# Fahien/rayca

Hardware: AMD Instinct MI355X
Metric: Mrays/sec (primary+shadow), 1920x1080 Sponza 1spp (higher is better)
Workload: dtype f32; 1 GPU; sponza-STAND-IN procedural atrium 271,568 tris, 1920x1080, primary + 1 shadow ray (Pathtracer max_depth=1, NEE, 1 point light), 1 spp; width=1920, height=1080, triangles=271568, bvh_nodes=135379, bvh_built_on=gpu (bvh_build.hip; same tree as the host builder), rays_per_frame=4146938, frames_in_flight=4, tiling=rows in bands of 8 dealt over 1 rank(s), frame_gather=none, launched_by=single process

## Files before the change

__graft_entry__.py:

```python
from __future__ import annotations

import os
import subprocess
import sys

ROOT = os.path.dirname(os.path.abspath(__file__))
CSRC = os.path.join(ROOT, "rayca_amd", "csrc")
LIB = os.path.join(CSRC, "librayca_hip.so")
HIPCC = os.environ.get("HIPCC", "/opt/rocm/bin/hipcc")

COMMON = ["-O3", "-std=c++17", "-fPIC", "-ffp-contract=off", "-fno-fast-math", "-Wall", "-Wno-unused-function",
          "-Wno-unused-result"]


def _stale(target, sources):
    if not os.path.exists(target):
        return True
    t = os.path.getmtime(target)
    return any(os.path.getmtime(s) > t for s in sources)


def build(force: bool = False) -> None:
    srcs = [os.path.join(CSRC, f) for f in ("kernels.hip", "refill.hip", "refill.hpp", "flavour.hpp", "trace_core.inc", "bvh_build.hip", "api.inc", "select.inc", "scene.inc", "post.inc", "aux_kernels.inc", "general.inc", "wavefront.inc", "surface.inc", "image_pass.inc", "denoise.inc", "denoise_variance.inc", "temporal.inc", "upsample.inc", "tonemap.inc",
                                            "host_scene.cpp", "host_scene.hpp", "device_types.hpp", "no_pk.hpp", "rayca_math.hpp", "staging.hpp", "libm_exact.hpp")]
    srcs.append(os.path.join(ROOT, "include", "rayca_hip.h"))
    if force or _stale(LIB, srcs):
        host_obj = os.path.join(CSRC, "host_scene.o")
        jobs = [subprocess.Popen(["g++", *COMMON, "-c", os.path.join(CSRC, "host_scene.cpp"), "-o", host_obj, "-pthread"])]
        objs = []
        for unit in ("kernels", "refill", "bvh_build"):
            obj = os.path.join(CSRC, unit + ".o")
            objs.append(obj)
            jobs.append(subprocess.Popen([HIPCC, "--offload-arch=gfx950", *COMMON, "-c", os.path.join(CSRC, unit + ".hip"), "-o", obj]))
        failed = [j.args for j in jobs if j.wait() != 0]
        if failed:
            raise subprocess.CalledProcessError(1, failed[0])
        subprocess.run([HIPCC, "--offload-arch=gfx950", "-shared", "-fPIC", *objs, host_obj, "-o", LIB, "-lpthread"], check=True)
    subprocess.run(["make", "-s", "-C", os.path.join(ROOT, "oracle")], check=True)
    build_cpp_host()
    build_cpp_host("resident_draw")
    build_microbench()
    if ROOT not in sys.path:
        sys.path.insert(0, ROOT)
    import rayca_amd
    from rayca_amd import abi, lib
    l = lib.load()
    for sym in abi.PRODUCT_SYMBOLS:
        getattr(l, sym)


def build_microbench() -> None:
    out_dir = os.path.join(ROOT, "tests", "microbench", "_build")
    os.makedirs(out_dir, exist_ok=True)
    for name, extra, deps in (("peaks", [], []), ("libm_compare", ["-ffp-contract=off", "-fno-fast-math"], [os.path.join(CSRC, "libm_exact.hpp")])):
        src, exe = os.path.join(ROOT, "tests", "microbench", name + ".hip"), os.path.join(out_dir, name)
        if _stale(exe, [src] + deps):
            subprocess.run([HIPCC, "--offload-arch=gfx950", "-O3", "-std=c++17", *extra, src, "-o", exe], check=True)


def build_cpp_host(program: str = "host_mirror") -> str:
    out_dir = os.path.join(ROOT, "tests", "cpp", "_build")
    exe = os.path.join(out_dir, program)
    srcs = [os.path.join(ROOT, "tests", "cpp", program + ".cpp"), os.path.join(ROOT, "include", "rayca.hpp"),
            os.path.join(ROOT, "include", "rayca_gltf.hpp"), os.path.join(ROOT, "include", "rayca_sdtf.hpp"), os.path.join(ROOT, "include", "rayca_jpeg.hpp"), os.path.join(ROOT, "include", "rayca_hip.h"), LIB]
    if _stale(exe, srcs):
        os.makedirs(out_dir, exist_ok=True)
        subprocess.run(["g++", "-std=c++17", "-O1", "-ffp-contract=off", "-Wall", "-Wextra", "-I" + os.path.join(ROOT, "include"), srcs[0], "-o", exe,
                        "-L" + CSRC, "-lrayca_hip", "-Wl,-rpath,$ORIGIN/../../../rayca_amd/csrc"], check=True)
    return exe


def smoke() -> None:
    if ROOT not in sys.path:
        sys.path.insert(0, ROOT)
    sys.path.insert(0, os.path.join(ROOT, "tests"))
    import numpy as np
    import torch

    assert torch.cuda.is_available(), "smoke() needs a GPU"
    build()
    import oracle_lib
    from rayca_amd import Config, DeviceScene, IntegratorStrategy, flatten, scenes

    desc = flatten(scenes.box_scene())
    ds = DeviceScene(desc, Config())
    orc = oracle_lib.OracleScene(desc, Config())
    for cfg in (Config(integrator=IntegratorStrategy.Flat), Config(max_depth=1)):
        u8, f32, st = ds.render(cfg, 64, 64)
        ou8, of32, _ = orc.render(cfg, 64, 64)
        assert (f32[..., 3] == 1.0).all()
        err = float((np.abs(f32 - of32) / np.maximum(1.0, np.abs(of32))).max())
        assert err <= 1e-4, f"smoke parity failed: max diff {err}"
        assert int(np.abs(u8.astype(int) - ou8.astype(int)).max()) <= 1
    from rayca_amd import abi
    desc = flatten(scenes.cornell_scene())
    ds2 = DeviceScene(desc, Config(), builder=abi.BUILDER_SAH)
    orc2 = oracle_lib.OracleScene(desc, Config())
    for cfg in (Config(integrator=IntegratorStrategy.Flat), Config(max_depth=1)):
        u8, f32, st = ds2.render(cfg, 96, 54)
        ou8, of32, _ = orc2.render(cfg, 96, 54)
        err = float((np.abs(f32 - of32) / np.maximum(1.0, np.abs(of32))).max())
        assert err <= 1e-4, f"smoke parity (SAH scene) failed: max diff {err}"
        assert int(np.abs(u8.astype(int) - ou8.astype(int)).max()) <= 1
    ds.close()
    ds2.close()
    print("smoke ok:", st)


if __name__ == "__main__":
    build(force="--force" in sys.argv)
    print("built", LIB)
```

rayca_amd/csrc/api.inc:

```
#include <dlfcn.h>

#include <algorithm>
#include <atomic>
#include <chrono>
#include <condition_variable>
#include <functional>
#include <memory>
#include <cstdio>
#include <cstdlib>
#include <cstring>
#include <mutex>
#include <string>
#include <thread>
#include <vector>

#include "refill.hpp"
#include "staging.hpp"

using namespace rayca;

namespace {

thread_local std::string g_last_error;

// ... 285 lines not shown
  uint32_t n = 0;
  for (uint32_t y = 0; y < height; ++y)
    if ((y / band) % t.parts == t.part) ++n;
  return n;
}

float quad_area(F4 ab, F4 ac) {
  const float ab_len = length(ab), ac_len = length(ac);
  const float cos_theta = dot(ab, ac) / (ab_len * ac_len);
  const float sin_theta = 1.0f - cos_theta;
  return sin_theta * ab_len * ac_len;
}

bool is_emissive(const RaycaMaterial& m) {
  if (m.kind != RAYCA_MATERIAL_PHONG) return false;
  const bool close_to_black = fabsf(m.emission[0] - 0.0f) < FLT_EPSILON && fabsf(m.emission[1] - 0.0f) < FLT_EPSILON &&
                              fabsf(m.emission[2] - 0.0f) < FLT_EPSILON && fabsf(m.emission[3] - 1.0f) < FLT_EPSILON;
  return !close_to_black;
}

DevMaterial dev_material(const RaycaMaterial& m) {
  DevMaterial d;
  std::memset(&d, 0, sizeof d);
  std::memcpy(d.color, m.color, 16); std::memcpy(d.ambient, m.ambient, 16); std::memcpy(d.emission, m.emission, 16);
  std::memcpy(d.diffuse, m.diffuse, 16); std::memcpy(d.specular, m.specular, 16);
  d.kind = m.kind; d.albedo_texture = m.albedo_texture; d.normal_texture = m.normal_texture;
  d.metallic_roughness_texture = m.metallic_roughness_texture;
  d.metallic_factor = m.metallic_factor; d.roughness_factor = m.roughness_factor; d.shininess = m.shininess;
  d.emissive = is_emissive(m) ? 1u : 0u;
  return d;
}

DevLight dev_light(const HostLight& l) {
  DevLight d;
  std::memset(&d, 0, sizeof d);
  d.kind = l.kind; d.material = l.material; d.intensity = l.intensity;
  d.color[0] = l.color.r; d.color[1] = l.color.g; d.color[2] = l.color.b; d.color[3] = l.color.a;
  d.attenuation[0] = l.attenuation.x; d.attenuation[1] = l.attenuation.y; d.attenuation[2] = l.attenuation.z;
  d.ab[0] = l.ab.x; d.ab[1] = l.ab.y; d.ab[2] = l.ab.z;
  d.ac[0] = l.ac.x; d.ac[1] = l.ac.y; d.ac[2] = l.ac.z;
  const F4 pos = to_point(trs_world_translation(l.local));
  d.position[0] = pos.x; d.position[1] = pos.y; d.position[2] = pos.z; d.position[3] = pos.w;
  const F4 dir = -rotate(vec3(1.0f, 0.0f, 0.0f), l.local.rotation);
  d.direction[0] = dir.x; d.direction[1] = dir.y; d.direction[2] = dir.z;
  d.trs_translation[0] = l.local.translation.x; d.trs_translation[1] = l.local.translation.y; d.trs_translation[2] = l.local.translation.z;
  d.trs_rotation[0] = l.local.rotation.x; d.trs_rotation[1] = l.local.rotation.y; d.trs_rotation[2] = l.local.rotation.z; d.trs_rotation[3] = l.local.rotation.w;
  d.trs_scale[0] = l.local.scale.x; d.trs_scale[1] = l.local.scale.y; d.trs_scale[2] = l.local.scale.z;
  if (l.kind == RAYCA_LIGHT_QUAD) {
    const F4 n = normalized(cross(l.ab, l.ac));
    d.normal[0] = n.x; d.normal[1] = n.y; d.normal[2] = n.z;
    d.area = quad_area(l.ab, l.ac);
  }
  return d;
}

#include "select.inc"


struct LaunchLog {
  FrameCtx* c = nullptr;
  size_t ev_used = 0;
  std::vector<int> ev_class;
  uint32_t launches = 0, trace_launches = 0;
};
template <typename Launch>
int32_t timed_launch(LaunchLog& log, hipStream_t stream, int cls, bool timed, bool trace, Launch&& launch, size_t* pair = nullptr) {
  std::vector<hipEvent_t>& ev = log.c->ev_trace;
  if (timed) {
    for (hipEvent_t e; ev.size() < log.ev_used + 2;) {
      HIP_TRY(hipEventCreate(&e));
      ev.push_back(e);
    }
    HIP_TRY(hipEventRecord(ev[log.ev_used], stream));
    log.ev_class.push_back(cls);
    if (pair) *pair = log.ev_used;
    log.ev_used += 2;
  }
  const int32_t rc = launch();
  if (rc != RAYCA_OK) return rc;
  HIP_TRY(hipGetLastError());
  if (timed) HIP_TRY(hipEventRecord(ev[log.ev_used - 1], stream));
  ++log.launches;
  if (trace) ++log.trace_launches;
  return RAYCA_OK;
}

struct ContextPass {
  FrameCtx* c;
  hipStream_t stream;
  void* record_event;
  bool timing;
  bool own_stream;
};
int32_t pass_acquire(RaycaScene* s, const RaycaRenderOptions& o, bool timing, ContextPass& p) {
  FrameCtx* c = &s->ctx[o.context];
  HIP_TRY(hipSetDevice(s->device));
  const int32_t rc = ensure_ctx(s, c);
  if (rc != RAYCA_OK) return rc;
  p = ContextPass{c, o.stream ? static_cast<hipStream_t>(o.stream) : c->stream, o.record_event, timing, o.stream == nullptr};
  if (c->frame_pending) HIP_TRY(hipStreamWaitEvent(p.stream, c->ev_done, 0));
  if (o.wait_event) HIP_TRY(hipStreamWaitEvent(p.stream, static_cast<hipEvent_t>(o.wait_event), 0));
  return RAYCA_OK;
}
int32_t pass_retire(const ContextPass& p) {
  if (p.timing) HIP_TRY(hipEventRecord(p.c->ev_end, p.stream));
  HIP_TRY(hipEventRecord(p.c->ev_done, p.stream));
  if (p.record_event) HIP_TRY(hipEventRecord(static_cast<hipEvent_t>(p.record_event), p.stream));
  p.c->frame_pending = true;
  return RAYCA_OK;
}
int32_t pass_finish(const ContextPass& p, uint32_t launches, RaycaStats* stats_out) {
  if (p.own_stream || stats_out) HIP_TRY(hipStreamSynchronize(p.stream));
  if (!stats_out) return RAYCA_OK;
  std::memset(stats_out, 0, sizeof *stats_out);
  HIP_TRY(hipEventElapsedTime(&stats_out->kernel_ms, p.c->ev_begin, p.c->ev_end));
  stats_out->kernel_launches = launches;
  stats_out->class_ms[RAYCA_KERNEL_OTHER] = stats_out->kernel_ms;
  stats_out->class_launches[RAYCA_KERNEL_OTHER] = launches;
  return RAYCA_OK;
}

constexpr int32_t kPassNothing = 1;
template <typename Prepare, typename Body>
int32_t run_pass(RaycaScene* s, const RaycaRenderOptions& o, RaycaStats* stats_out, Prepare&& prepare, Body&& body) {
  FrameCtx* c = &s->ctx[o.context];
  std::lock_guard<std::mutex> lock(c->mu);
  int32_t rc = prepare(c);
  if (rc != RAYCA_OK) return rc == kPassNothing ? RAYCA_OK : rc;
  ContextPass pass{};
  if ((rc = pass_acquire(s, o, stats_out != nullptr, pass)) != RAYCA_OK) return rc;
  if (pass.timing) HIP_TRY(hipEventRecord(c->ev_begin, pass.stream));
  uint32_t launches = 0;
  if ((rc = body(pass.stream, launches)) != RAYCA_OK) return rc;
  if ((rc = pass_retire(pass)) != RAYCA_OK) return rc;
  return pass_finish(pass, launches, stats_out);
}
template <typename Body>
int32_t run_pass(RaycaScene* s, const RaycaRenderOptions& o, RaycaStats* stats_out, Body&& body) {
  return run_pass(s, o, stats_out, [](FrameCtx*) -> int32_t { return RAYCA_OK; }, body);
}

enum : uint32_t { kOptTraversal = 1u, kOptCollectStats = 2u, kOptTile = 4u };
int32_t pass_options(const RaycaRenderOptions& o, const char* what, uint32_t accepts) {
  if (o.context >= kMaxContexts) return fail(RAYCA_ERR_BAD_ARG, "context out of range");
  if ((accepts & kOptTraversal) && o.traversal > RAYCA_TRAVERSAL_EXHAUSTIVE) return fail(RAYCA_ERR_BAD_ARG, "unknown traversal");
  const char* field = nullptr;
  if (!(accepts & kOptTraversal) && o.traversal != 0) field = "traversal";
  else if (!(accepts & kOptCollectStats) && o.collect_stats != 0) field = "collect_stats";
  else if (o.engine != 0) field = "engine";
  else if (o.camera_rays != 0) field = "camera_rays";
  else if (o.reserved != 0) field = "reserved";
  else if (!(accepts & kOptTile) && (o.tile.part != 0 || o.tile.parts != 0 || o.tile.band_rows != 0 || o.tile.reserved != 0)) field = "tile";
  if (field) return fail(RAYCA_ERR_BAD_ARG, std::string("RaycaRenderOptions.") + field + " does not apply to " + what + ": must be zero");
  return RAYCA_OK;
}

struct TuneEvent { int cls; size_t ev; int format; int refill; };

struct Frame {
  RaycaScene* s;
  FrameCtx* c;
  RaycaConfig cfg;
  RaycaRenderOptions opts;
  LaunchPlan plan;
  FrameParams fp;
  PathBuffers pb;
  hipStream_t stream;
  const DevScene* dscene;
  uint8_t* rgba8;
  float4* rgba32f;
  const RaycaRadiance* rays;
  uint32_t in_flight;
  bool fused;
  bool timing;
  bool all_formats;
  uint32_t node_format;
  int frame_format[2] = {-2, -2};
  bool frame_calibrates[2] = {false, false};
  std::vector<TuneEvent> tune_events;
  LaunchLog log;
};

struct GenQueues {
  QueuedRay* in;
  uint32_t* in_count;
  QueuedRay* out;
  uint32_t* out_count;
};

int32_t wavefront_generation(Frame& f, uint32_t g, const GenQueues& q) {
  RaycaScene* s = f.s;
  FrameCtx* c = f.c;
  const bool sph = s->host.sphere_count != 0, fast = s->dev.ref_leaf_of != nullptr, stats = f.plan.stats;
  const bool gen0 = g == 0 && !f.rays;
  if (fast)
    f.node_format |= gen0 ? ((RAYCA_WF_PRIMARY_WIDE ? 1u : 0u) | (RAYCA_WF_PRIMARY_HALF ? 4u : 0u)) : ((RAYCA_WF_BOUNCE_WIDE ? 2u : 0u) | (RAYCA_WF_BOUNCE_HALF ? 8u : 0u));
  const StackPlan sp = plan_stack(std::max(s->host.max_depth, s->host.max_depth4), RAYCA_WF_LDS_ENTRIES);
  const Trav trav = !fast ? kTravExact : (sp.spill_entries ? kTravFastSpill : kTravFast);
  const uint32_t npix = f.pb.npix;
  const uint32_t batches = gen0 ? f.fp.tile_count : (npix + 63u) / 64u;
  const uint32_t grid = (batches + 3u) / 4u;
  const uint32_t nls = (f.plan.mode == kModePath && f.cfg.direct_sampler == RAYCA_SAMPLER_NEE) ? (uint32_t)s->host.lights.size() * f.cfg.light_samples : 0u;
  int32_t rc;
  WfBuffers wb{};
  if ((rc = ensure(c->wf_hits, (size_t)npix * 16u)) != RAYCA_OK) return rc;
  wb.hits = static_cast<float4*>(c->wf_hits.ptr);
  wb.nls = nls;
  if (nls) {
    if ((rc = ensure(c->wf_sh_ray, (size_t)npix * nls * 32u)) != RAYCA_OK) return rc;
    if ((rc = ensure(c->wf_sh_x, (size_t)npix * nls * 16u)) != RAYCA_OK) return rc;
    wb.sh_ray = static_cast<float4*>(c->wf_sh_ray.ptr);
    wb.sh_x = static_cast<float4*>(c->wf_sh_x.ptr);
  }
  const bool wf_refill = knobs().wf_refill;
  const int shadow_refill_mode = knobs().wf_shadow_refill;
  TraceLaunch tl{};
  uint32_t lgrid = grid;
  const bool caller_rays = f.rays && g == 0;
  bool refill = (wf_refill || caller_rays) && !gen0 && fast;
  if (refill && (rc = persistent_grid(s, queue_refill_kernel(sph, stats, caller_rays), sp.lds_bytes, batches, true, f.in_flight, 0u, lgrid)) != RAYCA_OK) return rc;
  if ((rc = bind_stack(c, sp, lgrid, tl)) != RAYCA_OK) return rc;
  if (refill) tl.ticket = 1u;
  WfTraceKernel kt = pick_wf_trace(gen0, trav, sph, stats);
  rc = timed_launch(f.log, f.stream, refill ? RAYCA_KERNEL_QUEUE_REFILL : RAYCA_KERNEL_WF_TRACE, f.timing, true, [&] {
    if (refill)
      launch_queue_refill(sph, stats, caller_rays, lgrid, sp.lds_bytes, f.stream, *f.dscene, q.in, q.in_count, wb.hits, c->heads, c->counters, tl);
    else
      hipLaunchKernelGGL(kt, dim3(lgrid), dim3(kBlock), sp.lds_bytes, f.stream, *f.dscene, f.fp, q.in, q.in_count, wb, c->counters, tl);
    return RAYCA_OK;
  });
  if (rc != RAYCA_OK) return rc;
  WfShadeKernel ks = pick_wf_shade(f.plan.mode, gen0, f.fused, sph, caller_rays);
  const uint32_t shade_grid = ((gen0 ? f.fp.tile_count * 64u : npix) + kShadeBlock - 1) / kShadeBlock;
  rc = timed_launch(f.log, f.stream, RAYCA_KERNEL_WF_SHADE, f.timing, false, [&] {
    hipLaunchKernelGGL(ks, dim3(shade_grid), dim3(kShadeBlock), 0, f.stream, *f.dscene, f.fp, q.in, q.in_count, q.out, q.out_count, wb, f.pb, g,
                       f.rgba8, f.rgba32f, c->shade_stats);
    return RAYCA_OK;
  });
  if (rc != RAYCA_OK || !nls) return rc;
  lgrid = grid;
  refill = wf_refill && fast && (!gen0 ? shadow_refill_mode >= 1 : shadow_refill_mode >= 2);
  if (refill && (rc = persistent_grid(s, shadow_refill_kernel(gen0, sph, stats), sp.lds_bytes, batches, true, f.in_flight, 0u, lgrid)) != RAYCA_OK) return rc;
  if ((rc = bind_stack(c, sp, lgrid, tl)) != RAYCA_OK) return rc;
  if (refill) tl.ticket = 1u;
  WfShadowKernel kh = pick_wf_shadow(gen0, trav, sph, stats);
  const ShadowRefillArgs sa{wb.sh_ray, wb.sh_x, wb.nls, f.pb.direct, f.pb.state, f.pb.npix};
  return timed_launch(f.log, f.stream, refill ? RAYCA_KERNEL_SHADOW_REFILL : RAYCA_KERNEL_WF_SHADOW, f.timing, true, [&] {
    if (refill)
      launch_shadow_refill(gen0, sph, stats, lgrid, sp.lds_bytes, f.stream, *f.dscene, f.fp, q.in, q.in_count, sa, g, c->heads_b, c->counters, tl);
    else
      hipLaunchKernelGGL(kh, dim3(lgrid), dim3(kBlock), sp.lds_bytes, f.stream, *f.dscene, f.fp, q.in, q.in_count, wb, f.pb, g, c->counters, tl);
    return RAYCA_OK;
  });
}

GenChoice choose_generation(Frame& f, uint32_t g) {
  RaycaScene* s = f.s;
  const LaunchPlan& plan = f.plan;
  RaycaScene::Tune& tu = s->tune[plan.mode == kModePath ? 1 : 0][g == 0 ? 0 : 1];
  GenChoice ch{f.all_formats ? format_forced() : 0, false, false, false};
  const int refill_env = knobs().refill;
  const bool refill_possible = f.fused && plan.mode == kModeFlat && plan.ordered && s->dev.ref_leaf_of != nullptr;
  const int refill_forced = !refill_possible ? 0 : (f.opts.camera_rays == RAYCA_CAMERA_REFILL ? 1 : (f.opts.camera_rays == RAYCA_CAMERA_GENERATION ? 0 : refill_env));
  ch.refill = refill_forced > 0;
  bool kernel_pending = false;
  if (refill_possible && f.all_formats && refill_forced < 0) {
    std::lock_guard<std::mutex> tune_lock(s->tune_mu);
    if (tu.refill >= 0) ch.refill = tu.refill != 0;
    else if (f.pb.npix >= 65536u && !plan.stats && tu.refill_launched < 8u) {
      ch.refill = (tu.refill_launched++ & 1u) != 0;
      ch.refill_cal = true;
      if (ch.format < 0) ch.format = 1;
    } else {
      kernel_pending = true;
    }
  }
  const bool can_tune = plan.ordered && s->dev.ref_leaf_of != nullptr && wide_forced() < 0 && f.all_formats;
  if (can_tune && !ch.refill_cal && !kernel_pending) {
    const int cls = g == 0 ? 0 : 1;
    if (f.frame_format[cls] == -2) {
      std::lock_guard<std::mutex> tune_lock(s->tune_mu);
      f.frame_format[cls] = -1;
      if (tu.decided >= 0) f.frame_format[cls] = tu.decided;
      else if (f.pb.npix >= 65536u && !plan.stats && tu.launched < 16u) {
        f.frame_format[cls] = (int)(tu.launched++ & 3u);
        f.frame_calibrates[cls] = true;
      }
    }
    if (f.frame_format[cls] >= 0) ch.format = f.frame_format[cls];
    ch.calibrating = f.frame_calibrates[cls];
  }
  return ch;
}

int32_t fused_generation(Frame& f, uint32_t g, const GenQueues& q) {
  RaycaScene* s = f.s;
  FrameCtx* c = f.c;
  const GenChoice ch = choose_generation(f, g);
  const bool park = RAYCA_PARK_CTX && f.plan.mode == kModePath;
  const TravPlan tp = plan_traversal(s, f.plan.ordered, g, ch.format, park ? path_lds_entries() : kMaxLdsEntries);
  f.node_format |= (traits(tp.trav).wide ? (g == 0 ? 1u : 2u) : 0u) | (traits(tp.trav).half ? (g == 0 ? 4u : 8u) : 0u) | (ch.calibrating ? 256u : 0u) |
                   (ch.refill_cal ? 512u : 0u) | (ch.refill ? 1024u : 0u);
  const StackPlan sp = tp.stack;
  const size_t lds_bytes = sp.lds_bytes + (park ? (size_t)kCtxQuads * 16u * kBlock : 0u);
  const bool sph = s->host.sphere_count != 0;
  GenKernel k = pick_kernel(f.plan.mode, g == 0, f.fused, tp.trav, sph, f.plan.stats);
  const RefillFlavour rf{tp.trav, sph, f.plan.stats};
  const uint32_t batches = g == 0 ? f.fp.tile_count : (f.pb.npix + 63u) / 64u;
  const uint32_t grid_mult = knobs().grid_mult;
  uint32_t grid = 0;
  TraceLaunch tl{};
  int32_t rc = persistent_grid(s, ch.refill ? flat_refill_kernel(rf) : reinterpret_cast<const void*>(k), lds_bytes, batches, true, f.in_flight, grid_mult, grid);
  if (rc != RAYCA_OK || (rc = bind_stack(c, sp, grid, tl)) != RAYCA_OK) return rc;
  const uint32_t ticket_forced = knobs().ticket;
  tl.ticket = ticket_forced ? ticket_forced : (batches >= 16u * grid ? 2u : 1u);
  size_t ev = 0;
  rc = timed_launch(f.log, f.stream, ch.refill ? RAYCA_KERNEL_FLAT_REFILL : RAYCA_KERNEL_GENERATION, f.timing || ch.calibrating || ch.refill_cal, true, [&] {
    if (ch.refill)
      launch_flat_refill(rf, grid, lds_bytes, f.stream, *f.dscene, f.fp, c->heads, f.rgba8, f.rgba32f, c->counters, tl);
    else
      hipLaunchKernelGGL(k, dim3(grid), dim3(kBlock), lds_bytes, f.stream, *f.dscene, f.fp, c->heads, q.in, q.in_count, q.out, q.out_count, f.pb, g,
                         f.rgba8, f.rgba32f, c->counters, tl);
    return RAYCA_OK;
  }, &ev);
  if (rc != RAYCA_OK) return rc;
  if (ch.calibrating) f.tune_events.push_back({g == 0 ? 0 : 1, ev, ch.format, -1});
  if (ch.refill_cal) f.tune_events.push_back({0, ev, ch.format, ch.refill ? 1 : 0});
  return RAYCA_OK;
}

int32_t stack_machine(Frame& f) {
  RaycaScene* s = f.s;
  FrameCtx* c = f.c;
  const RaycaConfig& cfg = f.cfg;
  GeneralKernel k = pick_general_kernel(s->dev.ref_leaf_of != nullptr, s->host.sphere_count != 0, f.plan.stats);
  const StackPlan sp = plan_stack(s->host.max_depth);
  uint32_t grid = 0;
  int32_t rc = persistent_grid(s, reinterpret_cast<const void*>(k), sp.lds_bytes, f.fp.tile_count, false, 1u, 0u, grid);
  if (rc != RAYCA_OK) return rc;
  uint32_t levels = 1;
  if (cfg.integrator == RAYCA_INTEGRATOR_PATHTRACER) levels = cfg.russian_roulette ? 64u : (cfg.max_depth ? cfg.max_depth : 1u);
  else if (cfg.integrator == RAYCA_INTEGRATOR_RAYTRACER || cfg.integrator == RAYCA_INTEGRATOR_SCRATCHER) levels = cfg.max_depth + 2u;
  if (levels > 256u) return fail(RAYCA_ERR_UNSUPPORTED, "max_depth too large for the path-vertex stack");
  GFrameStore store{};
  store.threads = grid * kBlock;
  store.levels = levels + 1u;
  if ((rc = ensure(c->frames, (size_t)store.levels * 8u * store.threads * 16u)) != RAYCA_OK) return rc;
  store.frames = static_cast<float4*>(c->frames.ptr);
  if (cfg.direct_sampler == RAYCA_SAMPLER_MIS) {
    if ((rc = ensure(c->mis_samples, (size_t)2u * kMisMaxSamples * store.threads * 16u)) != RAYCA_OK) return rc;
    store.samples = static_cast<float4*>(c->mis_samples.ptr);
  }
  TraceLaunch tl{};
  if ((rc = bind_stack(c, sp, grid, tl)) != RAYCA_OK) return rc;
  tl.ticket = f.fp.tile_count >= 16u * grid ? 2u : 1u;
  c->heads_clean = false;
  return timed_launch(f.log, f.stream, RAYCA_KERNEL_OTHER, f.timing, true, [&]() -> int32_t {
    HIP_TRY(hipMemsetAsync(c->heads, 0, 8 * kHeadStride * sizeof(uint32_t), f.stream));
    hipLaunchKernelGGL(k, dim3(grid), dim3(kBlock), sp.lds_bytes, f.stream, s->dev, f.fp, c->heads, f.pb, store, c->counters, tl);
    return RAYCA_OK;
  });
}
int32_t stack_machine_status(Frame& f) {
  HIP_TRY(hipStreamSynchronize(f.stream));
  TraceCounters tc{};
  HIP_TRY(hipMemcpy(&tc, f.c->counters, sizeof tc, hipMemcpyDeviceToHost));
  if (tc.flags & kFlagTooDeep) return fail(RAYCA_ERR_UNSUPPORTED, "path recursion deeper than the path-vertex stack (Russian roulette did not terminate within 64 bounces)");
  if (tc.flags & kFlagUnsupported)
    return fail(RAYCA_ERR_UNSUPPORTED, "this Config reaches a todo!()/panic arm of the reference on this scene (e.g. directional light under NEE, quad light under Raytracer/Scratcher, get_t of a Pbr material, Whitted radiance of a Ggx material)");
  return RAYCA_OK;
}

int32_t resolve(Frame& f) {
  FrameCtx* c = f.c;
  const bool general = f.plan.mode == kModeGeneral;
  const int32_t rc = timed_launch(f.log, f.stream, RAYCA_KERNEL_OTHER, f.timing, false, [&] {
    hipLaunchKernelGGL(k_resolve, dim3((f.pb.npix + kBlock - 1) / kBlock), dim3(kBlock), 0, f.stream, f.fp, f.pb, f.plan.generations,
                       static_cast<float4*>(c->accum.ptr), f.rgba8, f.rgba32f, general ? nullptr : c->heads_b, 17u * kHeadStride);
    return RAYCA_OK;
  });
  if (rc == RAYCA_OK && !general) c->heads_clean = true;
  return rc;
}

int32_t book_calibration(Frame& f) {
  RaycaScene* s = f.s;
  HIP_TRY(hipStreamSynchronize(f.stream));
  float sum[2] = {0.0f, 0.0f};
  int fmt[2] = {-1, -1};
  int refill_choice = -1;
  float refill_ms = 0.0f;
  for (const TuneEvent& te : f.tune_events) {
    float ms = 0.0f;
    HIP_TRY(hipEventElapsedTime(&ms, f.c->ev_trace[te.ev], f.c->ev_trace[te.ev + 1]));
    if (te.refill >= 0) {
      refill_choice = te.refill;
      refill_ms = ms;
      continue;
    }
    sum[te.cls] += ms;
    fmt[te.cls] = te.format;
  }
  std::lock_guard<std::mutex> tune_lock(s->tune_mu);
  if (refill_choice >= 0) {
    RaycaScene::Tune& tu = s->tune[0][0];
    if (refill_ms < tu.refill_best[refill_choice]) tu.refill_best[refill_choice] = refill_ms;
    if (++tu.refill_booked == 8u) tu.refill = tu.refill_best[1] < tu.refill_best[0] ? 1 : 0;
  }
  for (int cls = 0; cls < 2; ++cls) {
    if (fmt[cls] < 0) continue;
    RaycaScene::Tune& tu = s->tune[f.plan.mode == kModePath ? 1 : 0][cls];
    if (sum[cls] < tu.best[fmt[cls] & 3]) tu.best[fmt[cls] & 3] = sum[cls];
    if (++tu.booked == 16u) {
      int pick = 0;
      for (int p = 1; p < 4; ++p)
        if (tu.best[p] < tu.best[pick]) pick = p;
      tu.decided = pick;
    }
  }
  return RAYCA_OK;
}

int32_t fill_stats(Frame& f, RaycaStats* out) {
  FrameCtx* c = f.c;
  const bool general = f.plan.mode == kModeGeneral;
  HIP_TRY(hipStreamSynchronize(f.stream));
  TraceCounters tc{};
  HIP_TRY(hipMemcpy(&tc, c->counters, sizeof tc, hipMemcpyDeviceToHost));
  if (f.plan.wavefront && !general) {
    std::vector<unsigned long long> lines(64 * 16);
    HIP_TRY(hipMemcpy(lines.data(), c->shade_stats, lines.size() * sizeof(unsigned long long), hipMemcpyDeviceToHost));
    for (size_t l = 0; l < 64; ++l) {
      tc.shaded += lines[l * 16 + 0];
      tc.shadow += lines[l * 16 + 1];
      tc.bounce += lines[l * 16 + 2];
    }
  }
  std::memset(out, 0, sizeof *out);
  out->rays_primary = (uint64_t)f.pb.npix * f.cfg.samples_per_pixel;
  out->rays_shadow = tc.shadow;
  out->rays_bounce = tc.bounce;
  out->boxes_tested = tc.boxes;
  out->triangles_tested = tc.tris;
  out->hits_shaded = tc.shaded;
  out->wave_box_slots = tc.box_slots;
  out->wave_triangle_slots = tc.tri_slots;
  static const bool nee_report = getenv("RAYCA_NEE_SKIP_REPORT") != nullptr;
  if (nee_report && f.plan.mode == kModePath && !f.plan.wavefront && f.plan.stats) fprintf(stderr, "[rayca nee] irrelevant %llu of %llu samples, skip %s\n", tc.nee_irrelevant, tc.shadow, f.fp.nee_skip ? "on" : "off");
  HIP_TRY(hipEventElapsedTime(&out->kernel_ms, c->ev_begin, c->ev_end));
  float tsum = 0.0f;
  for (size_t i = 0; i + 1 < f.log.ev_used; i += 2) {
    float ms = 0.0f;
    HIP_TRY(hipEventElapsedTime(&ms, c->ev_trace[i], c->ev_trace[i + 1]));
    const int cls = i / 2 < f.log.ev_class.size() ? f.log.ev_class[i / 2] : RAYCA_KERNEL_OTHER;
    out->class_ms[cls] += ms;
    out->class_launches[cls] += 1u;
    if (cls != RAYCA_KERNEL_WF_SHADE && (cls != RAYCA_KERNEL_OTHER || general)) tsum += ms;
  }
  out->trace_kernel_ms = tsum;
  out->kernel_launches = f.log.launches;
  out->trace_kernel_launches = f.log.trace_launches;
  out->rows_rendered = f.fp.rows;
  out->node_format = f.node_format;
  return RAYCA_OK;
}

int32_t camera_frame_params(const RaycaScene* s, uint32_t width, uint32_t height, const RaycaTile& tile_in, FrameParams& fp) {
  RaycaTile tile = tile_in;
  if (tile.parts == 0) { tile.parts = 1; tile.part = 0; }
  if (tile.part >= tile.parts) return fail(RAYCA_ERR_BAD_ARG, "tile.part >= tile.parts");
  if (tile.band_rows == 0) tile.band_rows = 1;
  const uint32_t rows = tile_rows(tile, height);
  fp.width = width; fp.height = height; fp.rows = rows;
  fp.part = tile.part; fp.parts = tile.parts; fp.band = tile.band_rows;
  fp.tiles_x = (width + kTileW - 1u) / kTileW;
  fp.tile_count = fp.tiles_x * ((rows + kTileH - 1u) / kTileH);
  const float fw = (float)width, fh = (float)height;
  fp.inv_width = 1.0f / fw;
  fp.inv_height = 1.0f / fh;
  fp.aspect = fw / fh;
  fp.angle = tanf(s->host.camera_yfov * 0.5f);
  fp.camera = s->host.world_trs[s->host.camera_node];
  return RAYCA_OK;
}
void camera_sample_params(uint32_t spp, uint32_t sample, FrameParams& fp) {
  const float strate = sqrtf((float)spp);
  const float sub_offset = 0.5f / strate, sub_step = 1.0f / strate;
  const uint32_t sc_i = (uint32_t)strate;
  const float ix = (float)(sample % sc_i), iy = (float)(sample / sc_i);
  fp.sample = sample;
  fp.sub_step_x = ix * sub_step;
  fp.sub_step_y = iy * sub_step;
  fp.sub_offset = sub_offset;
}

void config_frame_params(const Frame& f, FrameParams& fp) {
  const RaycaConfig& cfg = f.cfg;
  fp.integrator = cfg.integrator; fp.direct_sampler = cfg.direct_sampler; fp.indirect_sampler = cfg.indirect_sampler;
  fp.light_samples = cfg.light_samples; fp.light_stratify = cfg.light_stratify;
  fp.strate_count = cfg.light_stratify ? (uint32_t)sqrtf((float)cfg.light_samples) : 1u;
  fp.max_depth = cfg.max_depth; fp.russian_roulette = cfg.russian_roulette; fp.seed = cfg.seed; fp.spp = cfg.samples_per_pixel;
  fp.inv_gamma = 1.0f / cfg.gamma;
  fp.nee_skip = f.s->nee_skip && f.plan.ordered && !(f.dscene->root_ref & kLeafFlag) ? 1u : 0u;
}


int32_t frame_begin(Frame& f, const ContextPass& pass, void* d_rgba8, void* d_rgba32f) {
  RaycaScene* s = f.s;
  FrameCtx* c = f.c = f.log.c = pass.c;
  const LaunchPlan& plan = f.plan;
  f.stream = pass.stream;
  f.timing = pass.timing;
  int32_t rc;
  if ((plan.wavefront || format_forced() > 0) && (rc = formats_wait(s)) != RAYCA_OK) return rc;
  f.all_formats = formats_ready(s);
  f.dscene = f.all_formats ? &s->dev_full : &s->dev;
  f.in_flight = frames_in_flight_hint(s, f.opts.context, f.opts.stream != nullptr);
  f.node_format = (f.all_formats ? 0u : 2048u) | (RAYCA_NODE_CH && RAYCA_NODE_CH48 && f.dscene->nodes_ch ? 4096u : 0u);
  f.rgba8 = static_cast<uint8_t*>(d_rgba8);
  f.rgba32f = static_cast<float4*>(d_rgba32f);
  f.fused = f.cfg.samples_per_pixel == 1 && plan.mode == kModeFlat;
  config_frame_params(f, f.fp);

  PathBuffers& pb = f.pb;
  const uint32_t npix = pb.npix = f.fp.rows * f.fp.width;
  const size_t records = (size_t)npix * (plan.generations ? plan.generations : 1);
  const bool path = plan.mode == kModePath, bounces = path && plan.generations > 1;
  if (!f.fused) {
    if ((rc = ensure(c->path_direct, records * 16)) != RAYCA_OK) return rc;
    if ((rc = ensure(c->path_state, records * 4)) != RAYCA_OK) return rc;
    if (path && (rc = ensure(c->path_brdf, records * 16)) != RAYCA_OK) return rc;
    if (f.cfg.samples_per_pixel > 1 && (rc = ensure(c->accum, (size_t)npix * 16)) != RAYCA_OK) return rc;
    pb.direct = static_cast<float4*>(c->path_direct.ptr);
    pb.brdf = static_cast<float4*>(c->path_brdf.ptr);
    pb.state = static_cast<uint32_t*>(c->path_state.ptr);
  }
  if (bounces && (rc = ensure(c->queue[0], (size_t)npix * sizeof(QueuedRay))) != RAYCA_OK) return rc;
  if ((bounces || f.rays) && (rc = ensure(c->queue[1], (size_t)npix * sizeof(QueuedRay))) != RAYCA_OK) return rc;
  return RAYCA_OK;
}

int32_t frame_run(Frame& f) {
  FrameCtx* c = f.c;
  const hipStream_t stream = f.stream;
  const LaunchPlan& plan = f.plan;
  const bool general = plan.mode == kModeGeneral;
  const uint32_t npix = f.pb.npix, depths = plan.generations, spp = f.cfg.samples_per_pixel;
  int32_t rc;
  if (f.timing || general) HIP_TRY(hipMemsetAsync(c->counters, 0, kCountersBytes, stream));
  if (f.timing) HIP_TRY(hipEventRecord(c->ev_begin, stream));
  uint32_t* q_count = c->heads + 8 * kHeadStride;
  for (uint32_t sample = 0; sample < spp; ++sample) {
    if (!f.rays) camera_sample_params(spp, sample, f.fp);
    if (!f.fused && depths > 1) HIP_TRY(hipMemsetAsync(f.pb.state + npix, 0, (size_t)npix * (depths - 1) * 4, stream));
    if (general && (rc = stack_machine(f)) != RAYCA_OK) return rc;
    for (uint32_t g = 0; !general && g < depths; ++g) {
      if (!(g == 0 && c->heads_clean))
        HIP_TRY(hipMemsetAsync(c->heads_b, 0, (16 * kHeadStride + (g == 0 ? kHeadStride : 0)) * sizeof(uint32_t), stream));
      c->heads_clean = false;
      const int in = g ? (int)((g - 1) & 1) : (f.rays ? 1 : -1);
      const GenQueues q{in < 0 ? nullptr : static_cast<QueuedRay*>(c->queue[in].ptr), in < 0 ? nullptr : q_count + in,
                        static_cast<QueuedRay*>(c->queue[g & 1].ptr), q_count + (g & 1)};
      if (g != 0) HIP_TRY(hipMemsetAsync(q.out_count, 0, sizeof(uint32_t), stream));
      else if (f.rays) {
        const RaycaRadiance& rr = *f.rays;
        rc = timed_launch(f.log, stream, RAYCA_KERNEL_OTHER, f.timing, false, [&] {
          hipLaunchKernelGGL(k_enqueue_rays, dim3((npix + kBlock - 1u) / kBlock), dim3(kBlock), 0, stream, static_cast<const float*>(rr.rays), npix, rr.first_index,
                             f.cfg.seed, rr.sample, q.in, q.in_count);
          return RAYCA_OK;
        });
        if (rc != RAYCA_OK) return rc;
      }
      if ((rc = plan.wavefront ? wavefront_generation(f, g, q) : fused_generation(f, g, q)) != RAYCA_OK) return rc;
    }
    if (!f.fused && (rc = resolve(f)) != RAYCA_OK) return rc;
  }
  return RAYCA_OK;
}

int32_t frame_finish(Frame& f, const ContextPass& pass, RaycaStats* stats_out, bool caller_drains) {
  int32_t rc = pass_retire(pass);
  if (rc != RAYCA_OK) return rc;
  if (!f.tune_events.empty() && (rc = book_calibration(f)) != RAYCA_OK) return rc;
  if (f.plan.mode == kModeGeneral && (rc = stack_machine_status(f)) != RAYCA_OK) return rc;
  if (f.timing) return fill_stats(f, stats_out);
  return caller_drains ? RAYCA_OK : pass_finish(pass, f.log.launches, nullptr);
}

int32_t render_body(RaycaScene* s, const RaycaConfig* cfg_in, uint32_t width, uint32_t height, const RaycaRenderOptions* opts_in,
                    void* d_rgba8, void* d_rgba32f, RaycaStats* stats_out, bool caller_drains) {
  if (!s || !cfg_in) return fail(RAYCA_ERR_BAD_ARG, "null scene or config");
  if (width == 0 || height == 0) return fail(RAYCA_ERR_BAD_ARG, "empty image");
  if (!s->host.has_camera) return fail(RAYCA_ERR_NO_CAMERA, "scene has no camera (scene.rs:109)");
  if (const int32_t e = refuse_empty_scene(s); e != RAYCA_OK) return e;
  Frame f{};
  f.s = s;
  const RaycaConfig& cfg = f.cfg = *cfg_in;
  const RaycaRenderOptions& opts = f.opts;
  if (opts_in) f.opts = *opts_in;
  LaunchPlan& plan = f.plan;
  plan.ordered = opts.traversal != RAYCA_TRAVERSAL_EXHAUSTIVE;
  plan.stats = opts.collect_stats != 0;
  int32_t rc = validate_config(s, cfg, opts.engine, plan);
  if (rc != RAYCA_OK) return rc;
  if (opts.camera_rays > RAYCA_CAMERA_REFILL) return fail(RAYCA_ERR_BAD_ARG, "unknown camera_rays choice");
  if ((rc = camera_frame_params(s, width, height, opts.tile, f.fp)) != RAYCA_OK) return rc;
  if (f.fp.rows == 0) {
    if (stats_out) std::memset(stats_out, 0, sizeof *stats_out);
    return RAYCA_OK;
  }
  if (opts.context >= kMaxContexts) return fail(RAYCA_ERR_BAD_ARG, "context out of range");
  ContextPass pass{};
  if ((rc = pass_acquire(s, opts, stats_out != nullptr, pass)) != RAYCA_OK) return rc;
  if ((rc = frame_begin(f, pass, d_rgba8, d_rgba32f)) != RAYCA_OK || (rc = frame_run(f)) != RAYCA_OK) return rc;
  return frame_finish(f, pass, stats_out, caller_drains);
}

int32_t render_impl(RaycaScene* s, const RaycaConfig* cfg, uint32_t width, uint32_t height, const RaycaRenderOptions* opts,
                    void* d_rgba8, void* d_rgba32f, RaycaStats* stats_out) {
  if (!s) return fail(RAYCA_ERR_BAD_ARG, "null scene or config");
  const uint32_t context = opts ? opts->context : 0u;
  if (context >= kMaxContexts) return fail(RAYCA_ERR_BAD_ARG, "context out of range");
  std::lock_guard<std::mutex> lock(s->ctx[context].mu);
  return render_body(s, cfg, width, height, opts, d_rgba8, d_rgba32f, stats_out, false);
}

}

namespace {

struct Rccl {
  using Comm = void*;
  int (*CommInitAll)(Comm*, int, const int*) = nullptr;
  int (*CommDestroy)(Comm) = nullptr;
  int (*GroupStart)() = nullptr;
  int (*GroupEnd)() = nullptr;
  int (*Send)(const void*, size_t, int, int, Comm, hipStream_t) = nullptr;
  int (*Recv)(void*, size_t, int, int, Comm, hipStream_t) = nullptr;
  const char* (*GetErrorString)(int) = nullptr;
  bool ok = false;
  std::string why;
  static constexpr int kUint8 = 1;
  Rccl() {
    void* h = nullptr;
    for (const char* name : {"librccl.so.1", "librccl.so", "/opt/rocm/lib/librccl.so.1"})
      if ((h = dlopen(name, RTLD_NOW | RTLD_GLOBAL)) != nullptr) break;
    if (!h) {
      const char* e = dlerror();
      why = std::string("librccl could not be opened: ") + (e ? e : "?");
      return;
    }
    auto sym = [&](const char* n) { return dlsym(h, n); };
    CommInitAll = reinterpret_cast<decltype(CommInitAll)>(sym("ncclCommInitAll"));
    CommDestroy = reinterpret_cast<decltype(CommDestroy)>(sym("ncclCommDestroy"));
    GroupStart = reinterpret_cast<decltype(GroupStart)>(sym("ncclGroupStart"));
    GroupEnd = reinterpret_cast<decltype(GroupEnd)>(sym("ncclGroupEnd"));
    Send = reinterpret_cast<decltype(Send)>(sym("ncclSend"));
    Recv = reinterpret_cast<decltype(Recv)>(sym("ncclRecv"));
    GetErrorString = reinterpret_cast<decltype(GetErrorString)>(sym("ncclGetErrorString"));
    ok = CommInitAll && CommDestroy && GroupStart && GroupEnd && Send && Recv && GetErrorString;
    if (!ok) why = "librccl lacks one of ncclCommInitAll / ncclGroupStart / ncclSend / ncclRecv";
  }
};
Rccl& rccl() {
  static Rccl r;
  return r;
}
#define RCCL_TRY(expr)                                                                                         \
  do {                                                                                                         \
    const int r__ = (expr);                                                                                    \
    if (r__ != 0) return fail(RAYCA_ERR_RCCL, std::string(#expr) + ": " + rccl().GetErrorString(r__));        \
  } while (0)

#include "aux_kernels.inc"

void multi_release(RaycaScene* s) {
  MultiCtx& m = s->multi;
  m.workers.clear();
  if (!m.comms.empty() && rccl().ok)
    for (void* c : m.comms)
      if (c) (void)rccl().CommDestroy(c);
  m.comms.clear();
  for (MultiFrame& f : m.frames) {
    for (size_t i = 0; i < f.done.size(); ++i) {
      if (i < m.devices.size()) (void)hipSetDevice(m.devices[i]);
      if (f.done[i]) (void)hipEventDestroy(f.done[i]);
    }
    f.done.clear();
    (void)hipSetDevice(s->device);
    if (f.gathered) (void)hipEventDestroy(f.gathered);
    f.gathered = nullptr;
    f.gathered_valid = false;
    if (f.gather.ptr) (void)hipFree(f.gather.ptr);
    if (f.frame.ptr) (void)hipFree(f.frame.ptr);
    f.gather = DeviceBuffer{};
    f.frame = DeviceBuffer{};
    f.pending = false;
    f.status = RAYCA_OK;
    f.error.clear();
  }
  (void)hipSetDevice(s->device);
  m.devices.clear();
  m.peer_enabled = false;
}

}

extern "C" {

uint32_t rayca_hip_version(void) { return RAYCA_ABI_VERSION; }

int32_t rayca_hip_selftest(void) {
  std::string err;
  int32_t rc = selftest_half_rounding(err);
  if (rc == RAYCA_OK) rc = selftest_device_layouts(err);
  if (rc == RAYCA_OK) rc = selftest_kernel_selection(err);
  return rc == RAYCA_OK ? RAYCA_OK : fail(rc, err);
}

int32_t rayca_hip_device_count(void) {
  int n = 0;
  if (hipGetDeviceCount(&n) != hipSuccess) return 0;
  return n;
}

void rayca_hip_last_error(char* buf, size_t len) {
  if (!buf || !len) return;
  std::snprintf(buf, len, "%s", g_last_error.c_str());
}

void rayca_hip_config_default(RaycaConfig* out) {
  if (!out) return;
  std::memset(out, 0, sizeof *out);
  out->bvh = 1;
  out->light_samples = 1;
  out->light_stratify = 0;
  out->samples_per_pixel = 1;
  out->russian_roulette = 0;
  out->direct_sampler = RAYCA_SAMPLER_NEE;
  out->indirect_sampler = RAYCA_SAMPLER_COSINE;
  out->integrator = RAYCA_INTEGRATOR_PATHTRACER;
  out->max_depth = 5;
  out->gamma = 1.0f;
}

uint32_t rayca_hip_tile_rows(const RaycaTile* tile, uint32_t height) {
  if (!tile) return height;
  return tile_rows(*tile, height);
}

}

#include "scene.inc"

extern "C" {

int32_t rayca_hip_render_device(RaycaScene* s, const RaycaConfig* cfg, uint32_t width, uint32_t height, const RaycaRenderOptions* opts,
                                void* d_rgba8_out, void* d_rgba32f_out, RaycaStats* stats_out) {
  return render_impl(s, cfg, width, height, opts, d_rgba8_out, d_rgba32f_out, stats_out);
}

int32_t rayca_hip_render(RaycaScene* s, const RaycaConfig* cfg, uint32_t width, uint32_t height, const RaycaRenderOptions* opts, uint8_t* rgba8_out,
                         float* rgba32f_out, RaycaStats* stats_out) {
  if (!s) return fail(RAYCA_ERR_BAD_ARG, "null scene");
  RaycaRenderOptions o{};
  if (opts) o = *opts;
  RaycaTile tile = o.tile;
  if (tile.parts == 0) { tile.parts = 1; tile.part = 0; }
  const uint32_t rows = tile_rows(tile, height);
  const size_t npix = (size_t)rows * width;
  HIP_TRY(hipSetDevice(s->device));
  int32_t rc;
  if (o.context >= kMaxContexts) return fail(RAYCA_ERR_BAD_ARG, "context out of range");
  FrameCtx* c = &s->ctx[o.context];
  std::lock_guard<std::mutex> lock(c->mu);
  static const bool lap_on = getenv("RAYCA_RENDER_TIMING") != nullptr;
  auto lap_t = std::chrono::steady_clock::now();
  auto lap = [&](const char* what) {
    if (!lap_on) return;
    const auto now = std::chrono::steady_clock::now();
    fprintf(stderr, "[rayca render] %-28s %8.2f ms\n", what, std::chrono::duration<float, std::milli>(now - lap_t).count());
    lap_t = now;
  };
  if ((rc = ensure_ctx(s, c)) != RAYCA_OK) return rc;
  lap("frame context");
  if (c->frame_pending) HIP_TRY(hipEventSynchronize(c->ev_done));
  if (rgba8_out && (rc = ensure(c->out8, npix * 4 + 16)) != RAYCA_OK) return rc;
  if (rgba32f_out && (rc = ensure(c->out32, npix * 16 + 16)) != RAYCA_OK) return rc;
  lap("staging buffers");
  rc = render_body(s, cfg, width, height, &o, rgba8_out ? c->out8.ptr : nullptr, rgba32f_out ? c->out32.ptr : nullptr, stats_out, true);
  if (rc != RAYCA_OK) return rc;
  lap("render_body (issue)");
  hipStream_t stream = o.stream ? static_cast<hipStream_t>(o.stream) : c->stream;
  if (lap_on) {
    HIP_TRY(hipStreamSynchronize(stream));
    lap("kernels done");
  }
  if (rgba8_out && npix) HIP_TRY(hipMemcpyAsync(rgba8_out, c->out8.ptr, npix * 4, hipMemcpyDeviceToHost, stream));
  if (rgba32f_out && npix) HIP_TRY(hipMemcpyAsync(rgba32f_out, c->out32.ptr, npix * 16, hipMemcpyDeviceToHost, stream));
  HIP_TRY(hipStreamSynchronize(stream));
  lap("copy out");
  return RAYCA_OK;
}

}

struct RaycaRenderer {
  std::mutex mu;
  RaycaBuildOptions opts{};
  RaycaScene* scene = nullptr;
  KeptDesc kept;
  bool invalidated = false;
  uint32_t last_action = RAYCA_NONE;
  float last_ms[RAYCA_DRAW_MS_COUNT] = {0, 0, 0, 0};
  uint64_t builds = 0, updates = 0, reuses = 0;
};

extern "C" {

int32_t rayca_hip_renderer_create(const RaycaBuildOptions* opts, RaycaRenderer** out) {
  if (!out) return fail(RAYCA_ERR_BAD_ARG, "null out pointer");
  *out = nullptr;
  RaycaBuildOptions o{};
  o.builder = RAYCA_BUILDER_SAH;
  if (opts) o = *opts;
  if (o.builder != RAYCA_BUILDER_REFERENCE && o.builder != RAYCA_BUILDER_SAH) return fail(RAYCA_ERR_BAD_ARG, "unknown builder");
  RaycaRenderer* r = new RaycaRenderer();
  r->opts = o;
  *out = r;
  return RAYCA_OK;
}

int32_t rayca_hip_renderer_draw(RaycaRenderer* r, const RaycaSceneDesc* desc, const RaycaConfig* cfg, uint32_t width, uint32_t height,
                                const RaycaRenderOptions* opts, uint8_t* rgba8_out, float* rgba32f_out, RaycaStats* stats_out, uint32_t* action_out) {
  if (action_out) *action_out = RAYCA_NONE;
  if (!r || !desc) return fail(RAYCA_ERR_BAD_ARG, "null renderer or descriptor");
  std::lock_guard<std::mutex> lock(r->mu);
  using clock = std::chrono::steady_clock;
  auto ms_since = [](clock::time_point t) { return std::chrono::duration<float, std::milli>(clock::now() - t).count(); };
  const bool use_bvh = cfg ? cfg->bvh != 0 : true;
  float ms[RAYCA_DRAW_MS_COUNT] = {0, 0, 0, 0};
  std::string err;
  uint32_t action = RAYCA_DRAW_REBUILT;
  SceneGraph graph;
  const auto t_compare = clock::now();
  if (r->scene && r->kept.valid && !r->invalidated) {
    if (const int32_t rc = desc_compare(r->kept.view, r->kept.bvh, &r->kept.graph, *desc, use_bvh, action, graph, err); rc != RAYCA_OK) return fail(rc, err);
  } else {
    if (const int32_t rc = desc_validate(*desc, err); rc != RAYCA_OK) return fail(rc, err);
    if (const int32_t rc = scene_graph_pass(*desc, graph, err); rc != RAYCA_OK) return fail(rc, err);
  }
  ms[RAYCA_DRAW_MS_COMPARE] = ms_since(t_compare);
  if (action == RAYCA_DRAW_UPDATED) {
    const auto t = clock::now();
    const int32_t rc = rayca_hip_scene_update(r->scene, desc);
    if (rc == RAYCA_ERR_UNSUPPORTED) action = RAYCA_DRAW_REBUILT;
    else if (rc != RAYCA_OK) return rc;
    else {
      r->kept.refresh(*desc, std::move(graph));
      r->updates++;
      ms[RAYCA_DRAW_MS_UPDATE] = ms_since(t);
    }
  }
  if (action == RAYCA_DRAW_REBUILT) {
    if (!graph.has_camera) return fail(RAYCA_ERR_NO_CAMERA, "scene has no camera (scene.rs:109)");
    const auto t = clock::now();
    KeptDesc fresh;
    std::thread copier([&] { fresh.assign(*desc, use_bvh, std::move(graph)); });
    RaycaScene* made = nullptr;
    const int32_t rc = rayca_hip_scene_create(desc, cfg, &r->opts, &made);
    const std::string create_err = g_last_error;
    copier.join();
    if (rc != RAYCA_OK) return fail(rc, create_err);
    if (r->scene) (void)rayca_hip_scene_destroy(r->scene);
    r->scene = made;
    r->kept = std::move(fresh);
    r->invalidated = false;
    r->builds++;
    ms[RAYCA_DRAW_MS_BUILD] = ms_since(t);
  }
  const auto t_render = clock::now();
  if (const int32_t rc = rayca_hip_render(r->scene, cfg, width, height, opts, rgba8_out, rgba32f_out, stats_out); rc != RAYCA_OK) return rc;
  ms[RAYCA_DRAW_MS_RENDER] = ms_since(t_render);
  if (action == RAYCA_DRAW_REUSED) r->reuses++;
  r->last_action = action;
  std::copy(ms, ms + RAYCA_DRAW_MS_COUNT, r->last_ms);
  if (action_out) *action_out = action;
  return RAYCA_OK;
}

int32_t rayca_hip_renderer_last_draw(const RaycaRenderer* cr, uint32_t* action_out, float* ms_out, uint64_t* counters_out) {
  if (!cr) return fail(RAYCA_ERR_BAD_ARG, "null renderer");
  RaycaRenderer* r = const_cast<RaycaRenderer*>(cr);
  std::lock_guard<std::mutex> lock(r->mu);
  if (action_out) *action_out = r->last_action;
  if (ms_out) std::copy(r->last_ms, r->last_ms + RAYCA_DRAW_MS_COUNT, ms_out);
  if (counters_out) {
    counters_out[RAYCA_DRAW_N_BUILDS] = r->builds;
    counters_out[RAYCA_DRAW_N_UPDATES] = r->updates;
    counters_out[RAYCA_DRAW_N_REUSES] = r->reuses;
    counters_out[RAYCA_DRAW_N_KEPT_BYTES] = r->kept.bytes();
  }
  return RAYCA_OK;
}

int32_t rayca_hip_renderer_scene(RaycaRenderer* r, RaycaScene** out) {
  if (!r || !out) return fail(RAYCA_ERR_BAD_ARG, "null renderer or out pointer");
  std::lock_guard<std::mutex> lock(r->mu);
  *out = r->scene;
  return RAYCA_OK;
}

int32_t rayca_hip_renderer_invalidate(RaycaRenderer* r) {
  if (!r) return fail(RAYCA_ERR_BAD_ARG, "null renderer");
  std::lock_guard<std::mutex> lock(r->mu);
  r->invalidated = true;
  return RAYCA_OK;
}

int32_t rayca_hip_renderer_destroy(RaycaRenderer* r) {
  if (!r) return RAYCA_OK;
  RaycaScene* scene = nullptr;
  {
    std::lock_guard<std::mutex> lock(r->mu);
    scene = r->scene;
    r->scene = nullptr;
  }
  delete r;
  return rayca_hip_scene_destroy(scene);
}

int32_t rayca_hip_scene_desc_compare(const RaycaSceneDesc* resident, uint32_t resident_bvh, const RaycaSceneDesc* next, uint32_t next_bvh,
                                     uint32_t* action_out) {
  if (action_out) *action_out = RAYCA_NONE;
  if (!resident || !next || !action_out) return fail(RAYCA_ERR_BAD_ARG, "null descriptor or out pointer");
  std::string err;
  if (const int32_t rc = desc_validate(*resident, err); rc != RAYCA_OK) return fail(rc, "resident: " + err);
  SceneGraph graph;
  uint32_t action = RAYCA_DRAW_REBUILT;
  if (const int32_t rc = desc_compare(*resident, resident_bvh != 0, nullptr, *next, next_bvh != 0, action, graph, err); rc != RAYCA_OK) return fail(rc, err);
  *action_out = action;
  return RAYCA_OK;
}


int32_t rayca_hip_rccl_status(void) { return rccl().ok ? RAYCA_OK : fail(RAYCA_ERR_RCCL, rccl().why); }

}

namespace {

std::vector<std::unique_lock<std::mutex>> lock_contexts(RaycaScene* const* scenes, uint32_t count, uint32_t context) {
  std::vector<RaycaScene*> order(scenes, scenes + count);
  std::sort(order.begin(), order.end(), [](const RaycaScene* a, const RaycaScene* b) { return std::less<const RaycaScene*>()(a, b); });
  std::vector<std::unique_lock<std::mutex>> locks;
  for (RaycaScene* sc : order) locks.emplace_back(sc->ctx[context].mu);
  return locks;
}

int32_t multi_validate(RaycaScene* const* scenes, uint32_t count, const RaycaMultiOptions& mo) {
  if (!scenes || count == 0) return fail(RAYCA_ERR_BAD_ARG, "null argument");
  if (count > 64) return fail(RAYCA_ERR_BAD_ARG, "more than 64 devices");
  if (mo.gather > RAYCA_GATHER_PEER_COPY) return fail(RAYCA_ERR_BAD_ARG, "unknown gather transport");
  if (mo.context >= kMaxContexts) return fail(RAYCA_ERR_BAD_ARG, "context out of range");
  for (uint32_t i = 0; i < count; ++i)
    if (!scenes[i]) return fail(RAYCA_ERR_BAD_ARG, "null scene");
  for (uint32_t i = 0; i < count; ++i)
    for (uint32_t j = i + 1; j < count; ++j) {
      if (scenes[i] == scenes[j]) return fail(RAYCA_ERR_BAD_ARG, "the same scene handle twice");
      if (mo.gather == RAYCA_GATHER_RCCL && scenes[i]->device == scenes[j]->device)
        return fail(RAYCA_ERR_BAD_ARG, "RCCL needs every part on its own device (two scenes share one)");
    }
  return RAYCA_OK;
}

void multi_drain(RaycaScene* const* scenes, uint32_t count, uint32_t context) {
  for (uint32_t i = 0; i < count; ++i) {
    if (hipSetDevice(scenes[i]->device) != hipSuccess) continue;
    if (scenes[i]->ctx[context].stream) (void)hipStreamSynchronize(scenes[i]->ctx[context].stream);
  }
  (void)hipSetDevice(scenes[0]->device);
  (void)hipGetLastError();
}

int32_t multi_issue(RaycaScene* const* scenes, uint32_t count, const RaycaConfig* cfg, uint32_t width, uint32_t height, const RaycaMultiOptions& mo,
                    void* rgba8_out, RaycaStats* stats_out, bool asynchronous) {
  if (!cfg || !rgba8_out) return fail(RAYCA_ERR_BAD_ARG, "null argument");
  if (width == 0 || height == 0) return fail(RAYCA_ERR_BAD_ARG, "empty image");
  const uint32_t band = mo.band_rows ? mo.band_rows : 8u;
  const uint32_t ctx = mo.context;
  RaycaScene* s0 = scenes[0];
  std::lock_guard<std::mutex> multi_lock(s0->multi_mu);
  std::vector<std::unique_lock<std::mutex>> ctx_locks = lock_contexts(scenes, count, ctx);

  std::vector<uint32_t> rows(count);
  uint32_t max_rows = 0;
  for (uint32_t i = 0; i < count; ++i) {
    rows[i] = tile_rows(RaycaTile{i, count, band, 0}, height);
    max_rows = std::max(max_rows, rows[i]);
  }
  MultiCtx& m = s0->multi;
  std::vector<int> devices(count);
  for (uint32_t i = 0; i < count; ++i) devices[i] = scenes[i]->device;
  if (m.devices != devices) {
    (void)hipSetDevice(s0->device);
    for (MultiFrame& old : m.frames)
      if (old.pending && old.gathered) (void)hipEventSynchronize(old.gathered);
    multi_release(s0);
    m.devices = devices;
    for (uint32_t i = 1; i < count; ++i) m.workers.emplace_back(new PartWorker());
  }
  MultiFrame& f = m.frames[ctx];
  if (f.done.size() != count) {
    f.done.assign(count, nullptr);
    for (uint32_t i = 0; i < count; ++i) {
      HIP_TRY(hipSetDevice(devices[i]));
      HIP_TRY(hipEventCreateWithFlags(&f.done[i], hipEventDisableTiming));
    }
  }
// ... 427 lines not shown
```

rayca_amd/csrc/kernels.hip:

```cpp
#include "no_pk.hpp"
RAYCA_NO_PK_BEGIN
#include <hip/hip_runtime.h>
#include "device_types.hpp"
RAYCA_NO_PK_END

namespace rayca {
namespace {

RAYCA_NO_PK_BEGIN
#include "trace_core.inc"

template <int MODE, bool GEN0, bool ORDERED, bool FUSED, bool FAST, bool SPH, bool WIDE, bool SPILL, bool STATS, bool HALF>
__global__ __launch_bounds__(kBlock, MODE == kModeFlat ? RAYCA_MIN_WAVES_FLAT : RAYCA_MIN_WAVES) void k_generation(DevScene sc, FrameParams fp, uint32_t* heads, const QueuedRay* in_rays,
                                                       const uint32_t* in_count, QueuedRay* out_rays, uint32_t* out_count,
                                                       PathBuffers pb, uint32_t depth, uint8_t* rgba8, float4* rgba32f,
                                                       TraceCounters* counters, TraceLaunch tl) {
  extern __shared__ uint32_t lds_stack[];
  NodeStack<SPILL> stack = make_stack<SPILL>(lds_stack, tl, rc_bid() * kBlock + rc_tid());
  float4* const ctx_slot = reinterpret_cast<float4*>(lds_stack + tl.lds_entries * kBlock) + rc_tid();
  constexpr bool PARK = RAYCA_PARK_CTX && MODE == kModePath;
  const uint32_t lane = __lane_id();
  const uint32_t home = xcc_id();
  WorkCursor wc{};
  const uint32_t total = GEN0 ? fp.tile_count : (*in_count + 63u) / 64u;
  LaneCounters cnt{};
  uint32_t n_shaded = 0, n_shadow = 0, n_bounce = 0;
  const bool collect_emissive = GEN0 ? true : (fp.direct_sampler == RAYCA_SAMPLER_NONE);
  const uint32_t nee_lights = (MODE == kModePath && fp.direct_sampler == RAYCA_SAMPLER_NEE) ? sc.light_count : 0u;

  for (;;) {
    const uint32_t batch = next_batch(heads, total, home, wc, tl.ticket);
    if (batch == RAYCA_NONE) break;
    bool live;
    uint32_t p = 0, key = 0;
    DRay ray;
    if (GEN0) {
      const uint32_t ty = batch / fp.tiles_x, tx = batch - ty * fp.tiles_x;
      const uint32_t x = tx * kTileW + (lane & (kTileW - 1u)), r = ty * kTileH + (lane >> RAYCA_TILE_W_LOG2);
      live = x < fp.width && r < fp.rows;
      const uint32_t y = ((r / fp.band) * fp.parts + fp.part) * fp.band + (r % fp.band);
      p = r * fp.width + x;
      if (live) {
        ray = camera_ray(fp, x, y);
        key = rng_root(fp.seed, y * fp.width + x, fp.sample);
      }
    } else {
      const uint32_t i = batch * 64u + lane;
      live = i < *in_count;
      if (live) {
        const QueuedRay q = in_rays[i];
        ray = make_ray(point3(q.ox, q.oy, q.oz), vec3(q.dx, q.dy, q.dz));
        p = q.pixel;
        key = q.key;
      }
    }
    const size_t slot = (size_t)depth * pb.npix + p;
    bool in_shadow = false;
    float t_stop = FLT_MAX;
    ShadeCtx cx;
    Color ns_x = black();
    Color direct = black();
    uint32_t li = 0, k = 0, dim = 0;
    const bool has_pixel = live;
    bool tail = false;

    while (live) {
      DHit hit;
      constexpr int kLeaveK = !ORDERED ? 0 : (MODE == kModeFlat ? RAYCA_LEAVE_K_CAMERA : (GEN0 ? RAYCA_LEAVE_K_PATH0 : RAYCA_LEAVE_K_BOUNCE));
      constexpr int kSlackForm = MODE == kModeFlat ? kSlackAlways : (GEN0 ? kSlackPerWave : kSlackNever);
      const bool found = trace<ORDERED, FAST, SPH, WIDE, SPILL, STATS, HALF, kLeaveK, kSlackForm>(sc, ray, t_stop, stack, hit, cnt);
      if (!in_shadow) {
        if (!found) {
          if (FUSED) direct = black() + black();
          else pb.state[slot] = kVertexNone;
          live = false;
        } else {
          n_shaded++;
          Color color;
          bool emissive;
          shade_hit<SPH>(sc, ray, hit, MODE == kModePath, color, emissive, cx);
          if (MODE == kModeFlat) {
            if (FUSED) direct = black() + color;
            else {
              pb.direct[slot] = as_f4(color);
              pb.state[slot] = kVertexEmissive;
            }
            live = false;
          } else if (collect_emissive && emissive) {
            pb.direct[slot] = as_f4(color);
            pb.state[slot] = kVertexEmissive;
            live = false;
          } else {
            in_shadow = true;
            if (PARK) {
              park_ctx(ctx_slot, cx);
              float zero = 0.0f;
              asm volatile("" : "+v"(zero));
              ctx_slot[6 * kBlock] = make_float4(zero, zero, zero, 1.0f);
            }
          }
        }
      } else {
        bool lit;
        if (t_stop == FLT_MAX) {
          lit = false;
          if (found) {
            const uint32_t hm = sc.ext[hit.prim].material;
            lit = hm != RAYCA_NONE && hm < sc.material_count && sc.materials[hm].emissive != 0u;
          }
        } else {
          lit = !(found && hit.t < t_stop);
        }
        if (PARK) {
          const Color sum = as_color(ctx_slot[6 * kBlock]) + (lit ? as_color(ctx_slot[5 * kBlock]) : black());
          ctx_slot[6 * kBlock] = as_f4(sum);
        } else {
          direct = direct + (lit ? ns_x : black());
        }
        if (++k == fp.light_samples) {
          k = 0;
          ++li;
        }
      }
      if (live && in_shadow) {
        bool pending = false;
        while (li < nee_lights) {
          if (PARK) cx = unpark_ctx(ctx_slot);
          const NeeSample ns = nee_prepare(sc, fp, cx, li, k, key, dim, ray);
          const bool irrelevant = ORDERED && nee_irrelevant(ns);
          if (STATS) {
            const unsigned long long m = __ballot(irrelevant);
            if (m != 0ull && lane == (uint32_t)__ffsll((long long)m) - 1u) atomicAdd(&counters->nee_irrelevant, (unsigned long long)__popcll(m));
          }
          if (irrelevant && fp.nee_skip) {
            if (++k == fp.light_samples) {
              k = 0;
              ++li;
            }
            continue;
          }
          if (PARK) ctx_slot[5 * kBlock] = as_f4(ns.x);
          else ns_x = ns.x;
          t_stop = ns.t_stop;
          pending = true;
          break;
        }
        if (!pending) {
          tail = true;
          live = false;
        }
      }
    }
    if (FUSED) {
      if (has_pixel) finalize_pixel(fp, direct, p, rgba8, rgba32f);
    } else if (MODE == kModePath) {
      bool want_bounce = false;
      QueuedRay next{};
      if (tail) {
        const uint32_t limit = fp.direct_sampler != RAYCA_SAMPLER_NONE ? fp.max_depth - 1u : fp.max_depth;
        const bool hemi = fp.indirect_sampler == RAYCA_SAMPLER_HEMISPHERE;
        F4 sdir = vec3(0.0f, 0.0f, 0.0f);
        if (depth < limit) {
          const float e1 = rng_f32(key, dim++), e2 = rng_f32(key, dim++);
          const float theta = hemi ? rc_acosf(e1) : rc_acosf(sqrtf(e1));
          const float omega_a = 2.0f * kPi * e2;
          const float st = rc_sinf(theta);
          sdir = vec3(rc_cosf(omega_a) * st, rc_sinf(omega_a) * st, rc_cosf(theta));
        }
        if (PARK) {
          cx = unpark_ctx(ctx_slot);
          direct = as_color(ctx_slot[6 * kBlock]);
        }
        pb.direct[slot] = as_f4(direct);
        if (depth < limit) {
          const F4 w = cx.normal;
          const F4 a = close(w, vec3(0, 1, 0)) ? vec3(1, 0, 0) : vec3(0, 1, 0);
          const F4 u = normalized(cross(a, w));
          F4 v = cross(w, u);
          if (hemi) v = normalized(v);
          const F4 omega_i = (sdir.x * u + sdir.y * v) + sdir.z * w;
          const Color brdf = surf_brdf(cx, omega_i);
          Color factor;
          if (hemi) factor = ((2.0f * kPi) * brdf) * clampf(dot(cx.normal, omega_i), 0.0f, 1.0f);
          else factor = kPi * brdf;
          pb.brdf[slot] = as_f4(factor);
          pb.state[slot] = kVertexLit;
          if (depth + 1u < fp.max_depth) {
            want_bounce = true;
            next.ox = cx.next_origin.x; next.oy = cx.next_origin.y; next.oz = cx.next_origin.z;
            next.dx = omega_i.x; next.dy = omega_i.y; next.dz = omega_i.z;
            next.pixel = p;
            next.key = rng_child(key, 0u);
          }
        } else {
          pb.state[slot] = kVertexLitNoIndirect;
        }
      }
      n_shadow += (uint32_t)__popcll(__ballot(tail)) * nee_lights * fp.light_samples;
      n_bounce += (uint32_t)__popcll(__ballot(want_bounce));
      push_ray(want_bounce, next, out_rays, out_count);
    }
  }
  if (STATS) {
    unsigned long long b = cnt.boxes, t = cnt.tris, sh = n_shaded, sb = cnt.slot_boxes, stt = cnt.slot_tris;
    for (int off = 32; off > 0; off >>= 1) {
      b += __shfl_down(b, off);
      t += __shfl_down(t, off);
      sh += __shfl_down(sh, off);
      sb += __shfl_down(sb, off);
      stt += __shfl_down(stt, off);
    }
    if (lane == 0) {
      atomicAdd(&counters->boxes, b);
      atomicAdd(&counters->tris, t);
      atomicAdd(&counters->shaded, sh);
      atomicAdd(&counters->box_slots, sb);
      atomicAdd(&counters->tri_slots, stt);
    }
  }
  if (MODE == kModePath) {
    const unsigned long long s2 = n_shadow, b2 = n_bounce;
    if (lane == 0 && (s2 | b2)) {
      atomicAdd(&counters->shadow, s2);
      atomicAdd(&counters->bounce, b2);
    }
  }
}

__global__ __launch_bounds__(kBlock) void k_resolve(FrameParams fp, PathBuffers pb, uint32_t depths, float4* accum, uint8_t* rgba8, float4* rgba32f,
                                                    uint32_t* clear, uint32_t clear_words) {
  if (clear && rc_bid() == 0)
    for (uint32_t i = rc_tid(); i < clear_words; i += rc_bdim()) clear[i] = 0u;
  const uint32_t p = rc_bid() * rc_bdim() + rc_tid();
  if (p >= pb.npix) return;
  bool some = false;
  Color L = black();
  for (int g = (int)depths - 1; g >= 0; --g) {
    const size_t slot = (size_t)g * pb.npix + p;
    const uint32_t st = pb.state[slot];
    if (st == kVertexNone) {
      some = false;
    } else if (st == kVertexEmissive) {
      some = true;
      L = as_color(pb.direct[slot]);
    } else {
      const Color direct = as_color(pb.direct[slot]);
      Color indirect = black();
      if (st == kVertexLit) {
        Color li = black();
        if (some) {
          const Color factor = as_color(pb.brdf[slot]);
          const Color x = (factor * L) * 1.0f;
          li = li + x;
        }
        indirect = indirect + li / (float)fp.light_samples;
      }
      L = direct + indirect;
      some = true;
    }
  }
  const Color c = some ? L : black();
  const Color prev = fp.sample == 0 ? black() : as_color(accum[p]);
  const Color acc = prev + c;
  if (fp.sample + 1u == fp.spp) finalize_pixel(fp, acc, p, rgba8, rgba32f);
  else accum[p] = as_f4(acc);
}

template <bool ORDERED, bool FAST, bool SPH, bool WIDE, bool SPILL, bool STATS>
__global__ __launch_bounds__(kBlock, RAYCA_TRACE_MIN_WAVES) void k_trace_rays(DevScene sc, const float* rays, uint32_t count, float* t_out, uint32_t* prim_out, float* uv_out,
                                                       TraceCounters* counters, TraceLaunch tl) {
  extern __shared__ uint32_t lds_stack[];
  NodeStack<SPILL> stack = make_stack<SPILL>(lds_stack, tl, rc_bid() * kBlock + rc_tid());
  const uint32_t i = rc_bid() * rc_bdim() + rc_tid();
  LaneCounters cnt{};
  if (i < count) {
    const float* r = rays + 6ull * i;
    const DRay ray = make_ray(point3(r[0], r[1], r[2]), vec3(r[3], r[4], r[5]));
    DHit hit;
    const bool found = trace<ORDERED, FAST, SPH, WIDE, SPILL, STATS, false, 0, kSlackAlways>(sc, ray, FLT_MAX, stack, hit, cnt);
    t_out[i] = found ? hit.t : FLT_MAX;
    prim_out[i] = found ? hit.prim : RAYCA_NONE;
    uv_out[2 * i] = found ? hit.u : 0.0f;
    uv_out[2 * i + 1] = found ? hit.v : 0.0f;
  }
  if (STATS) {
    unsigned long long b = cnt.boxes, t = cnt.tris;
    for (int off = 32; off > 0; off >>= 1) {
      b += __shfl_down(b, off);
      t += __shfl_down(t, off);
    }
    if (__lane_id() == 0) {
      atomicAdd(&counters->boxes, b);
      atomicAdd(&counters->tris, t);
    }
  }
}

template <bool ORDERED, bool FAST, bool SPH, bool WIDE, bool SPILL, bool STATS, bool OCCLUDED>
__global__ __launch_bounds__(kBlock, RAYCA_TRACE_MIN_WAVES) void k_query_rays(DevScene sc, QueryIo q, TraceCounters* counters, TraceLaunch tl) {
  extern __shared__ uint32_t lds_stack[];
  NodeStack<SPILL> stack = make_stack<SPILL>(lds_stack, tl, rc_bid() * kBlock + rc_tid());
  const uint32_t i = rc_bid() * rc_bdim() + rc_tid();
  LaneCounters cnt{};
  if (i < q.count) {
    bool dead;
    const float bound = query_bound(q, i, dead);
    DHit hit;
    hit.t = INFINITY;
    hit.prim = RAYCA_NONE;
    hit.u = hit.v = 0.0f;
    if (!dead) {
      const float* r = q.rays + 6ull * i;
      const DRay ray = make_ray(point3(r[0], r[1], r[2]), vec3(r[3], r[4], r[5]));
      const float t_stop = !OCCLUDED ? FLT_MAX : (bound < FLT_MAX ? bound : __uint_as_float(0x7F7FFFFEu));
      trace<ORDERED, FAST, SPH, WIDE, SPILL, STATS, false, 0, kSlackAlways>(sc, ray, t_stop, stack, hit, cnt);
    }
    query_store<OCCLUDED>(q, i, hit, query_found(hit, bound));
  }
  if (STATS) {
    unsigned long long b = cnt.boxes, t = cnt.tris;
    for (int off = 32; off > 0; off >>= 1) {
      b += __shfl_down(b, off);
      t += __shfl_down(t, off);
    }
    if (__lane_id() == 0) {
      atomicAdd(&counters->boxes, b);
      atomicAdd(&counters->tris, t);
    }
  }
}

#include "general.inc"
#include "wavefront.inc"
#include "surface.inc"
RAYCA_NO_PK_END
#include "image_pass.inc"
#include "denoise.inc"
#include "denoise_variance.inc"
#include "temporal.inc"
#include "upsample.inc"
#include "tonemap.inc"

}
}

#include "api.inc"
```

rayca_amd/csrc/select.inc:

```
#ifndef RAYCA_WF_LDS_ENTRIES
#define RAYCA_WF_LDS_ENTRIES 16u
#endif

struct LaunchPlan {
  int mode;
  bool ordered, stats;
  bool wavefront;
  uint32_t generations;
};



using GenKernel = void (*)(DevScene, FrameParams, uint32_t*, const QueuedRay*, const uint32_t*, QueuedRay*, uint32_t*, PathBuffers, uint32_t,
                           uint8_t*, float4*, TraceCounters*, TraceLaunch);
GenKernel pick_kernel(int mode, bool gen0, bool fused, Trav t, bool sph, bool stats) {
  const bool flat = mode == kModeFlat;
  return with_flavour([](auto T, auto FLAT, auto A, auto SPH, auto STATS) -> GenKernel {
    return k_generation<FLAT ? kModeFlat : kModePath, FLAT || A, T.ORDERED, FLAT && A, T.FAST, SPH, T.WIDE, T.SPILL, STATS, T.HALF>;
  }, t, flat, flat ? fused : gen0, sph, stats);
}

using TraceKernel = void (*)(DevScene, const float*, uint32_t, float*, uint32_t*, float*, TraceCounters*, TraceLaunch);
TraceKernel pick_trace_kernel(Trav t, bool sph, bool stats) {
  return with_flavour([](auto T, auto SPH, auto STATS) -> TraceKernel { return k_trace_rays<T.ORDERED, T.FAST, SPH, T.WIDE, T.SPILL, STATS>; }, t, sph, stats);
}

using QueryKernel = void (*)(DevScene, QueryIo, TraceCounters*, TraceLaunch);
QueryKernel pick_query_kernel(Trav t, bool sph, bool stats, bool occluded) {
  return with_flavour([](auto T, auto SPH, auto STATS, auto OCCLUDED) -> QueryKernel {
    return k_query_rays<T.ORDERED, T.FAST, SPH, false, true, STATS, T.ORDERED && OCCLUDED>;
  }, t, sph, stats, occluded);
}

using WfTraceKernel = void (*)(DevScene, FrameParams, const QueuedRay*, const uint32_t*, WfBuffers, TraceCounters*, TraceLaunch);
using WfShadowKernel = void (*)(DevScene, FrameParams, const QueuedRay*, const uint32_t*, WfBuffers, PathBuffers, uint32_t, TraceCounters*, TraceLaunch);
using WfShadeKernel = void (*)(DevScene, FrameParams, const QueuedRay*, const uint32_t*, QueuedRay*, uint32_t*, WfBuffers, PathBuffers, uint32_t, uint8_t*,
                               float4*, unsigned long long*);
WfTraceKernel pick_wf_trace(bool gen0, Trav t, bool sph, bool stats) {
  return with_flavour([](auto T, auto GEN0, auto SPH, auto STATS) -> WfTraceKernel { return k_wf_trace<GEN0, T.FAST, SPH, T.SPILL, STATS>; }, t, gen0, sph, stats);
}
WfShadowKernel pick_wf_shadow(bool gen0, Trav t, bool sph, bool stats) {
  return with_flavour([](auto T, auto GEN0, auto SPH, auto STATS) -> WfShadowKernel { return k_wf_shadow<GEN0, T.FAST, SPH, T.SPILL, STATS>; }, t, gen0, sph, stats);
}
WfShadeKernel pick_wf_shade(int mode, bool gen0, bool fused, bool sph, bool rays) {
  const bool flat = mode == kModeFlat;
  return with_flags([](auto FLAT, auto A, auto SPH, auto RAYS) -> WfShadeKernel {
    return k_wf_shade<FLAT ? kModeFlat : kModePath, !RAYS && (FLAT || A), FLAT && (RAYS || A), SPH, RAYS>;
  }, flat, flat ? fused : gen0, sph, rays);
}

using GeneralKernel = void (*)(DevScene, FrameParams, uint32_t*, PathBuffers, GFrameStore, TraceCounters*, TraceLaunch);
GeneralKernel pick_general_kernel(bool fast, bool sph, bool stats) {
  return with_flags([](auto FAST, auto SPH, auto STATS) -> GeneralKernel { return k_general<true, FAST, SPH, true, STATS>; }, fast, sph, stats);
}

using SurfaceKernel = void (*)(DevScene, SurfaceIo);
SurfaceKernel pick_surface_kernel(bool sph) {
  return with_flags([](auto SPH) -> SurfaceKernel { return k_surface<SPH>; }, sph);
}

#ifndef RAYCA_MAX_LDS_ENTRIES
#define RAYCA_MAX_LDS_ENTRIES 24
#endif
constexpr uint32_t kMaxLdsEntries = RAYCA_MAX_LDS_ENTRIES;
struct StackPlan {
  uint32_t lds_entries, spill_entries;
  size_t lds_bytes;
};
StackPlan plan_stack(uint32_t need, uint32_t max_entries = kMaxLdsEntries) {
  StackPlan p;
  const uint32_t want = need + 1u;
  p.lds_entries = want < max_entries ? ((want + 3u) / 4u) * 4u : max_entries;
  if (p.lds_entries == 0) p.lds_entries = 4;
  p.spill_entries = want > p.lds_entries ? want - p.lds_entries : 0u;
  p.lds_bytes = (size_t)p.lds_entries * kBlock * 4u;
  return p;
}
int32_t bind_stack(FrameCtx* c, const StackPlan& sp, uint32_t grid, TraceLaunch& tl) {
  tl = TraceLaunch{};
  tl.lds_entries = sp.lds_entries;
  if (sp.spill_entries) {
    tl.ovf_stride = grid * kBlock;
    const int32_t rc = ensure(c->stack_spill, (size_t)sp.spill_entries * tl.ovf_stride * 4u);
    if (rc != RAYCA_OK) return rc;
    tl.ovf = static_cast<uint32_t*>(c->stack_spill.ptr);
  }
  return RAYCA_OK;
}

#ifndef RAYCA_PATH_LDS_ENTRIES
#define RAYCA_PATH_LDS_ENTRIES 12
#endif
struct Knobs {
  int format;
  int wavefront;
  bool wf_refill;
  int wf_shadow_refill;
  int refill;
  uint32_t grid_mult;
  uint32_t ticket;
  uint32_t path_lds_entries;
};
const Knobs& knobs() {
  static const Knobs k = [] {
    const auto env = [](const char* name, int unset) { const char* e = getenv(name); return e ? atoi(e) : unset; };
    Knobs n{};
    n.format = getenv("RAYCA_NODE_FORMAT") ? env("RAYCA_NODE_FORMAT", 0) & 3 : (getenv("RAYCA_WIDE") ? (env("RAYCA_WIDE", 0) ? 1 : 0) : -1);
    n.wavefront = env("RAYCA_WAVEFRONT", -1);
    n.wf_refill = env("RAYCA_WF_REFILL", 1) != 0;
    n.wf_shadow_refill = env("RAYCA_WF_SHADOW_REFILL", 1);
    n.refill = getenv("RAYCA_REFILL") ? (env("RAYCA_REFILL", 0) != 0 ? 1 : 0) : -1;
    n.grid_mult = (uint32_t)env("RAYCA_GRID_MULT", 0);
    n.ticket = (uint32_t)env("RAYCA_TICKET", 0);
    n.path_lds_entries = std::min(std::max((uint32_t)env("RAYCA_PATH_LDS_ENTRIES", RAYCA_PATH_LDS_ENTRIES), 4u), kMaxLdsEntries);
    return n;
  }();
  return k;
}

int format_forced() { return knobs().format; }
int wide_forced() {
  const int f = format_forced();
  return f < 0 ? -1 : (f & 1);
}
bool use_wide(uint32_t generation) {
  const int forced = wide_forced();
  return forced >= 0 ? forced != 0 : generation > 0;
}
uint32_t path_lds_entries() { return knobs().path_lds_entries; }

struct TreeFacts {
  bool fast;
  bool formats;
  bool half_nodes;
  uint32_t depth, depth4;
};
struct TravPlan {
  Trav trav;
  StackPlan stack;
};
TravPlan plan_traversal(const TreeFacts& tf, bool ordered, uint32_t generation, int format_choice, uint32_t max_lds_entries) {
  TravPlan tp{};
  const bool fast = tf.fast;
  const bool wide = ordered && fast && tf.formats && (format_choice >= 0 ? (format_choice & 1) != 0 : use_wide(generation));
  const bool half = ordered && fast && format_choice >= 0 && (format_choice & 2) != 0 && tf.formats && tf.half_nodes;
  tp.stack = plan_stack(wide ? tf.depth4 : tf.depth, max_lds_entries);
  if (!ordered) tp.trav = fast ? kTravFastAll : kTravExactAll;
  else if (!fast) tp.trav = kTravExact;
  else if (wide) tp.trav = half ? kTravFastWideHalf : kTravFastWide;
  else if (tp.stack.spill_entries) tp.trav = half ? kTravFastSpillHalf : kTravFastSpill;
  else tp.trav = half ? kTravFastHalf : kTravFast;
  return tp;
}
TravPlan plan_traversal(const RaycaScene* s, bool ordered, uint32_t generation, int format_choice = -1, uint32_t max_lds_entries = kMaxLdsEntries) {
  const bool formats = formats_ready(s);
  const TreeFacts tf{s->dev.ref_leaf_of != nullptr, formats, formats && s->dev_full.nodes_h != nullptr, s->host.max_depth, s->host.max_depth4};
  return plan_traversal(tf, ordered, generation, format_choice, max_lds_entries);
}

bool wavefront_by_default(uint32_t generations) {
  const int forced = knobs().wavefront;
  if (forced >= 0) return forced != 0;
  return generations >= 3u;
}

const char* generation_kernels_gap(const RaycaConfig& c) {
  if (c.integrator == RAYCA_INTEGRATOR_FLAT) return nullptr;
  if (c.integrator != RAYCA_INTEGRATOR_PATHTRACER) return "integrator";
  if (c.russian_roulette) return "russian_roulette";
  if (c.direct_sampler != RAYCA_SAMPLER_NONE && c.direct_sampler != RAYCA_SAMPLER_NEE) return "direct_sampler";
  const uint32_t limit = c.direct_sampler != RAYCA_SAMPLER_NONE ? (c.max_depth ? c.max_depth - 1u : 0u) : c.max_depth;
  const bool bounces = limit > 0 && c.max_depth > 0;
  if (bounces) {
    if (c.indirect_sampler != RAYCA_SAMPLER_COSINE && c.indirect_sampler != RAYCA_SAMPLER_HEMISPHERE) return "indirect_sampler";
    if (c.light_samples != 1) return "light_samples";
  }
  return nullptr;
}
bool nee_meets_directional_light(const RaycaScene* s, const RaycaConfig& c) {
  if (c.integrator == RAYCA_INTEGRATOR_PATHTRACER && c.direct_sampler == RAYCA_SAMPLER_NEE)
    for (const HostLight& l : s->host.lights)
      if (l.kind == RAYCA_LIGHT_DIRECTIONAL) return true;
  return false;
}
bool generation_kernels_cover(const RaycaScene* s, const RaycaConfig& c) {
  return generation_kernels_gap(c) == nullptr && !nee_meets_directional_light(s, c);
}

int32_t refuse_empty_scene(const RaycaScene* s) {
  if (s->host.blas.empty() || s->prim_count == 0) return fail(RAYCA_ERR_EMPTY_SCENE, "empty TLAS (tlas.rs:272)");
  return RAYCA_OK;
}

int32_t validate_config(const RaycaScene* s, const RaycaConfig& c, uint32_t engine, LaunchPlan& plan) {
  if (c.samples_per_pixel == 0 || c.light_samples == 0) return fail(RAYCA_ERR_BAD_ARG, "samples_per_pixel and light_samples must be > 0");
  if (c.integrator > RAYCA_INTEGRATOR_PATHTRACER) return fail(RAYCA_ERR_BAD_ARG, "unknown integrator");
  if (c.direct_sampler > RAYCA_SAMPLER_MIS || c.indirect_sampler > RAYCA_SAMPLER_MIS) return fail(RAYCA_ERR_BAD_ARG, "unknown sampler");
  if (engine > RAYCA_ENGINE_FUSED) return fail(RAYCA_ERR_BAD_ARG, "unknown engine");
  const uint32_t generations_if_path = c.integrator == RAYCA_INTEGRATOR_PATHTRACER ? c.max_depth : 1u;
  plan.wavefront = plan.ordered && (engine == RAYCA_ENGINE_WAVEFRONT || (engine == RAYCA_ENGINE_AUTO && wavefront_by_default(generations_if_path)));
  if (c.integrator == RAYCA_INTEGRATOR_FLAT) {
    plan.mode = kModeFlat;
    plan.generations = 1;
    return RAYCA_OK;
  }
  if (engine == RAYCA_ENGINE_GENERAL || !generation_kernels_cover(s, c)) {
    if (!plan.ordered) return fail(RAYCA_ERR_UNSUPPORTED, "exhaustive traversal is only offered with the generation kernels");
    plan.mode = kModeGeneral;
    plan.generations = 1;
    return RAYCA_OK;
  }
  plan.mode = kModePath;
  plan.generations = c.max_depth;
  return RAYCA_OK;
}

int32_t kernel_registers(const void* k, uint32_t& regs) {
  static std::mutex mu;
  static std::vector<std::pair<const void*, uint32_t>> cache;
  std::lock_guard<std::mutex> lock(mu);
  for (const auto& e : cache)
    if (e.first == k) { regs = e.second; return RAYCA_OK; }
  hipFuncAttributes fa{};
  HIP_TRY(hipFuncGetAttributes(&fa, k));
  regs = fa.numRegs > 0 ? (uint32_t)fa.numRegs : 128u;
  cache.emplace_back(k, regs);
  return RAYCA_OK;
}

int32_t persistent_grid(const RaycaScene* s, const void* kernel, size_t lds_bytes, uint32_t batches, bool capped, uint32_t in_flight,
                        uint32_t per_cu_forced, uint32_t& grid) {
  uint32_t per_cu = per_cu_forced;
  if (per_cu == 0) {
    uint32_t regs = 0;
    const int32_t rc = kernel_registers(kernel, regs);
    if (rc != RAYCA_OK) return rc;
    per_cu = std::min(512u / (((regs + 7u) / 8u) * 8u), lds_bytes ? (uint32_t)((160u * 1024u) / lds_bytes) : 8u);
    if (capped) {
      per_cu = std::max(1u, std::min(per_cu, 8u));
      if (in_flight >= 4u) per_cu = (per_cu + 1u) / 2u;
      else if (in_flight >= 2u) per_cu = (per_cu * 3u + 3u) / 4u;
    }
    per_cu = std::max(1u, per_cu);
  }
  const uint32_t need = (batches + 3u) / 4u;
  grid = std::min((uint32_t)s->cu_count * per_cu, need ? need : 1u);
  return RAYCA_OK;
}

struct GenChoice {
  int format;
  bool calibrating;
  bool refill;
  bool refill_cal;
};

struct PickerFamily {
  const char* picker;
  std::vector<Trav> travs;
  int bits;
  std::function<const void*(Trav, uint32_t)> pick;
  std::function<uint32_t(Trav, uint32_t)> id;
};
int32_t check_family(const PickerFamily& f, std::string& err) {
  struct Picked { const void* kernel; uint32_t id; std::string tuple; };
  std::vector<Picked> v;
  for (Trav t : f.travs)
    for (uint32_t i = 0; i < (1u << f.bits); ++i) v.push_back({f.pick(t, i), f.id(t, i), "trav " + std::to_string(t) + ", flags " + std::to_string(i)});
  for (size_t i = 0; i < v.size(); ++i) {
    if (!v[i].kernel) { err = std::string(f.picker) + ": (" + v[i].tuple + ") gets no kernel"; return RAYCA_ERR_BAD_ARG; }
    for (size_t j = 0; j < i; ++j)
      if ((v[i].kernel == v[j].kernel) != (v[i].id == v[j].id)) {
        err = std::string(f.picker) + ": (" + v[j].tuple + ") and (" + v[i].tuple + (v[i].id == v[j].id ? ") must be one kernel and are two" : ") must be two kernels and are one");
        return RAYCA_ERR_BAD_ARG;
      }
  }
  return RAYCA_OK;
}
int32_t selftest_kernel_selection(std::string& err) {
  const auto b = [](uint32_t i, int n) { return (i >> n & 1u) != 0; };
  const auto P = [](auto kernel) { return reinterpret_cast<const void*>(kernel); };
  const auto mode = [](bool flat) { return flat ? kModeFlat : kModePath; };
  std::vector<Trav> all, none{kTravFast}, wf{kTravFast, kTravFastSpill, kTravExact}, fast{kTravFast, kTravFastSpill, kTravFastWide, kTravFastHalf, kTravFastSpillHalf, kTravFastWideHalf};
  for (int t = 0; t < kTravCount; ++t) all.push_back((Trav)t);
  const auto f32_of = [](Trav t) { return t == kTravFastHalf ? kTravFast : t == kTravFastSpillHalf ? kTravFastSpill : t == kTravFastWideHalf ? kTravFastWide : t; };
  const auto query_of = [](Trav t) { return t == kTravExact || t == kTravExactAll || t == kTravFastAll ? t : kTravFastSpill; };
  const auto exhaustive = [](Trav t) { return t == kTravExactAll || t == kTravFastAll; };
  const auto every = [](Trav t, uint32_t i) { return (uint32_t)t << 8 | i; };
  const PickerFamily families[] = {
      {"pick_kernel(trav; sph, stats, flat, gen0, fused)", all, 5,
       [&](Trav t, uint32_t i) { return P(pick_kernel(mode(b(i, 2)), b(i, 3), b(i, 4), t, b(i, 0), b(i, 1))); },
       [&](Trav t, uint32_t i) { return (uint32_t)t << 8 | (i & 7u) | ((b(i, 2) ? b(i, 4) : b(i, 3)) ? 8u : 0u); }},
      {"pick_trace_kernel(trav; sph, stats)", all, 2, [&](Trav t, uint32_t i) { return P(pick_trace_kernel(t, b(i, 0), b(i, 1))); },
       [&](Trav t, uint32_t i) { return (uint32_t)f32_of(t) << 8 | i; }},
      {"pick_query_kernel(trav; sph, stats, occluded)", all, 3, [&](Trav t, uint32_t i) { return P(pick_query_kernel(t, b(i, 0), b(i, 1), b(i, 2))); },
       [&](Trav t, uint32_t i) { return (uint32_t)query_of(t) << 8 | (i & 3u) | (!exhaustive(t) && b(i, 2) ? 4u : 0u); }},
      {"pick_wf_trace(trav; sph, stats, gen0)", wf, 3, [&](Trav t, uint32_t i) { return P(pick_wf_trace(b(i, 2), t, b(i, 0), b(i, 1))); }, every},
      {"pick_wf_shadow(trav; sph, stats, gen0)", wf, 3, [&](Trav t, uint32_t i) { return P(pick_wf_shadow(b(i, 2), t, b(i, 0), b(i, 1))); }, every},
      {"pick_wf_shade(sph, flat, rays, gen0, fused)", none, 5, [&](Trav, uint32_t i) { return P(pick_wf_shade(mode(b(i, 1)), b(i, 3), b(i, 4), b(i, 0), b(i, 2))); },
       [&](Trav, uint32_t i) { return (i & 7u) | (!b(i, 2) && (b(i, 1) ? b(i, 4) : b(i, 3)) ? 8u : 0u); }},
      {"pick_general_kernel(fast, sph, stats)", none, 3, [&](Trav, uint32_t i) { return P(pick_general_kernel(b(i, 0), b(i, 1), b(i, 2))); }, every},
      {"pick_surface_kernel(sph)", none, 1, [&](Trav, uint32_t i) { return P(pick_surface_kernel(b(i, 0))); }, every},
      {"flat_refill_kernel(trav; sph, stats)", fast, 2, [&](Trav t, uint32_t i) { return flat_refill_kernel(RefillFlavour{t, b(i, 0), b(i, 1)}); }, every},
      {"queue_refill_kernel(sph, stats, slack)", none, 3, [&](Trav, uint32_t i) { return queue_refill_kernel(b(i, 0), b(i, 1), b(i, 2)); }, every},
      {"query_refill_kernel(occluded, sph, stats)", none, 3, [&](Trav, uint32_t i) { return query_refill_kernel(b(i, 0), b(i, 1), b(i, 2)); }, every},
      {"shadow_refill_kernel(gen0, sph, stats)", none, 3, [&](Trav, uint32_t i) { return shadow_refill_kernel(b(i, 0), b(i, 1), b(i, 2)); }, every},
  };
  for (const PickerFamily& f : families)
    if (const int32_t rc = check_family(f, err); rc != RAYCA_OK) return rc;
  for (uint32_t i = 0; i < 64; ++i)
    for (int format_choice = -1; format_choice < 4; ++format_choice)
      for (uint32_t depth : {3u, 40u}) {
        const bool ordered = b(i, 0), generation = b(i, 5);
        const TreeFacts tf{b(i, 1), b(i, 2), b(i, 3), depth, b(i, 4) ? depth : depth / 2u + 1u};
        const TravPlan tp = plan_traversal(tf, ordered, generation, format_choice, kMaxLdsEntries);
        const TravTraits tr = traits(tp.trav);
        const bool wide = ordered && tf.fast && tf.formats && (format_choice >= 0 ? (format_choice & 1) != 0 : use_wide(generation));
        const bool half = ordered && tf.fast && tf.formats && tf.half_nodes && format_choice >= 0 && (format_choice & 2) != 0;
        const char* what = tr.ordered != ordered ? "ORDERED is not what was asked for" : tr.fast != tf.fast ? "FAST is not the scene's"
                         : tr.wide != wide ? "WIDE is not the node format asked for" : tr.half != half ? "HALF is not the node format asked for"
                         : tr.wide && !tr.spill ? "WIDE without SPILL" : tr.half && !(tr.ordered && tr.fast) ? "HALF without ORDERED and FAST"
                         : tp.stack.spill_entries && !tr.spill ? "a stack plan with spill entries for a flavour without SPILL" : nullptr;
        if (what) {
          err = std::string("plan_traversal(fast ") + std::to_string(tf.fast) + ", formats " + std::to_string(tf.formats) + ", half_nodes " + std::to_string(tf.half_nodes) +
                ", depth " + std::to_string(tf.depth) + ", depth4 " + std::to_string(tf.depth4) + "; ordered " + std::to_string(ordered) + ", generation " +
                std::to_string(generation) + ", format_choice " + std::to_string(format_choice) + ") gives flavour " + std::to_string(tp.trav) + ": " + what;
          return RAYCA_ERR_BAD_ARG;
        }
      }
  return RAYCA_OK;
}
```

rayca_amd/csrc/trace_core.inc:

```
constexpr int kBlock = 256;
#ifndef RAYCA_TRACE_MIN_WAVES
#define RAYCA_TRACE_MIN_WAVES 1
#endif
#ifndef RAYCA_MIN_WAVES_FLAT
#define RAYCA_MIN_WAVES_FLAT 5
#endif
#ifndef RAYCA_MIN_WAVES
#define RAYCA_MIN_WAVES 4
#endif

__device__ __forceinline__ uint32_t rc_tid() { return __builtin_amdgcn_workitem_id_x(); }
__device__ __forceinline__ uint32_t rc_bid() { return __builtin_amdgcn_workgroup_id_x(); }
__device__ __forceinline__ uint32_t rc_bdim() { return __builtin_amdgcn_workgroup_size_x(); }
__device__ __forceinline__ uint32_t rc_gdim() { return __builtin_amdgcn_grid_size_x() / __builtin_amdgcn_workgroup_size_x(); }

struct DRay {
  F4 o, d, rd;
};
struct DHit {
  float t;
  uint32_t prim;
  float u, v;
};

__device__ __forceinline__ DRay make_ray(F4 origin, F4 dir) {
  DRay r;
  r.rd = reciprocal(dir);
  origin.w = 1.0f;
  r.o = origin;
  r.d = dir;
  return r;
}

__device__ __forceinline__ bool slab(float ax, float ay, float az, float bx, float by, float bz, const DRay& r, float& tmin_out) {
  const float t1x = __fmaf_rn(ax - r.o.x, r.rd.x, 0.0f), t2x = __fmaf_rn(bx - r.o.x, r.rd.x, 0.0f);
  const float t1y = __fmaf_rn(ay - r.o.y, r.rd.y, 0.0f), t2y = __fmaf_rn(by - r.o.y, r.rd.y, 0.0f);
  const float t1z = __fmaf_rn(az - r.o.z, r.rd.z, 0.0f), t2z = __fmaf_rn(bz - r.o.z, r.rd.z, 0.0f);
  const float tmax = fminf(fminf(fmaxf(t1x, t2x), fmaxf(t1y, t2y)), fminf(fmaxf(t1z, t2z), FLT_MAX));
  const float tmin = fmaxf(fmaxf(fminf(t1x, t2x), fminf(t1y, t2y)), fmaxf(fminf(t1z, t2z), -FLT_MAX));
  tmin_out = tmin;
  return tmax >= tmin && tmax > 0.0f;
}

#ifndef RAYCA_RAY_SLACK
#define RAYCA_RAY_SLACK 1
#endif
struct FastRay {
  float mx, my, mz, cx, cy, cz;
#if RAYCA_RAY_SLACK
  float slack;
  bool fixed;
#endif
};
__device__ __forceinline__ bool fix_axis(float& m, float& c, float o, float centre, float inv_scale) {
  if (fabsf(c) <= FLT_MAX && fabsf(m) <= FLT_MAX) return false;
  const float d = centre - o;
  if (!(fabsf(d) <= FLT_MAX)) {
    m = 0.0f;
    c = -FLT_MAX;
    return true;
  }
  const float big = copysignf(fminf(1.2676506002282294e30f, 1.329227995784916e36f / fabsf(d)), m);
  m = big * inv_scale;
  c = d * big;
  return true;
}
__device__ __forceinline__ FastRay make_fast(const DevScene& sc, const DRay& r, bool half) {
  FastRay f;
  if (half) {
    f.mx = r.rd.x * sc.half_inv_scale; f.my = r.rd.y * sc.half_inv_scale; f.mz = r.rd.z * sc.half_inv_scale;
    f.cx = (sc.half_center[0] - r.o.x) * r.rd.x; f.cy = (sc.half_center[1] - r.o.y) * r.rd.y; f.cz = (sc.half_center[2] - r.o.z) * r.rd.z;
  } else {
    f.mx = r.rd.x; f.my = r.rd.y; f.mz = r.rd.z;
    f.cx = -(r.o.x * r.rd.x); f.cy = -(r.o.y * r.rd.y); f.cz = -(r.o.z * r.rd.z);
  }
#if RAYCA_RAY_SLACK
  f.fixed = fix_axis(f.mx, f.cx, r.o.x, half ? sc.half_center[0] : 0.0f, half ? sc.half_inv_scale : 1.0f);
  f.fixed |= fix_axis(f.my, f.cy, r.o.y, half ? sc.half_center[1] : 0.0f, half ? sc.half_inv_scale : 1.0f);
  f.fixed |= fix_axis(f.mz, f.cz, r.o.z, half ? sc.half_center[2] : 0.0f, half ? sc.half_inv_scale : 1.0f);
  f.slack = fmaxf(fmaxf(fabsf(f.cx), fabsf(f.cy)), fabsf(f.cz)) * 4.76837158203125e-07f;
#endif
  return f;
}
__device__ __forceinline__ bool ray_needs_slack(const DevScene& sc, const DRay& r, const FastRay& f) {
#if RAYCA_RAY_SLACK
  const float radius = sc.cull_abs * 4096.0f;
  return !(fabsf(r.o.x) <= radius && fabsf(r.o.y) <= radius && fabsf(r.o.z) <= radius) || f.fixed;
#else
  return false;
#endif
}
template <bool SLACK>
__device__ __forceinline__ bool slab_verdict(float tmin, float tmax, const FastRay& f) {
#if RAYCA_RAY_SLACK
  if (SLACK) {
    const float tp = tmax + f.slack;
    return tp >= tmin && tp > 0.0f;
  }
#endif
  return tmax >= tmin && tmax > 0.0f;
}
template <bool SLACK>
__device__ __forceinline__ float cull_limit(const DevScene& sc, const FastRay& f, float b) {
#if RAYCA_RAY_SLACK
  if (SLACK) return b + fabsf(b) * 9.765625e-4f + sc.cull_abs + f.slack;
#endif
  return b + fabsf(b) * 9.765625e-4f + sc.cull_abs;
}
typedef _Float16 rc_h2 __attribute__((ext_vector_type(2)));
__device__ __forceinline__ float lo16(uint32_t w) { return (float)__builtin_bit_cast(rc_h2, w).x; }
__device__ __forceinline__ float hi16(uint32_t w) { return (float)__builtin_bit_cast(rc_h2, w).y; }
template <bool SLACK>
__device__ __forceinline__ bool slab_fast(float ax, float ay, float az, float bx, float by, float bz, const FastRay& f, float& tmin_out) {
  const float t1x = __fmaf_rn(ax, f.mx, f.cx), t2x = __fmaf_rn(bx, f.mx, f.cx);
  const float t1y = __fmaf_rn(ay, f.my, f.cy), t2y = __fmaf_rn(by, f.my, f.cy);
  const float t1z = __fmaf_rn(az, f.mz, f.cz), t2z = __fmaf_rn(bz, f.mz, f.cz);
  const float tmax = fminf(fminf(fmaxf(t1x, t2x), fmaxf(t1y, t2y)), fmaxf(t1z, t2z));
  const float tmin = fmaxf(fmaxf(fminf(t1x, t2x), fminf(t1y, t2y)), fminf(t1z, t2z));
  tmin_out = tmin;
  return slab_verdict<SLACK>(tmin, tmax, f);
}
#ifndef RAYCA_NODE_CH
#define RAYCA_NODE_CH 1
#endif
#ifndef RAYCA_NODE_CH48
#define RAYCA_NODE_CH48 1
#endif
constexpr uint32_t kChNodeQuads = RAYCA_NODE_CH48 ? 3u : 4u;
constexpr uint32_t kChRefScale = RAYCA_NODE_CH48 ? 48u : 1u;
#ifndef RAYCA_WF_PRIMARY_WIDE
#define RAYCA_WF_PRIMARY_WIDE 0
#endif
#ifndef RAYCA_WF_PRIMARY_HALF
#define RAYCA_WF_PRIMARY_HALF 1
#endif
#ifndef RAYCA_WF_BOUNCE_WIDE
#define RAYCA_WF_BOUNCE_WIDE 1
#endif
#ifndef RAYCA_WF_BOUNCE_HALF
#define RAYCA_WF_BOUNCE_HALF 1
#endif
#ifndef RAYCA_WF_SHADOW_WIDE
#define RAYCA_WF_SHADOW_WIDE 1
#endif
#ifndef RAYCA_WF_SHADOW_HALF
#define RAYCA_WF_SHADOW_HALF 1
#endif
template <bool SLACK>
__device__ __forceinline__ bool slab_ch(float cx, float cy, float cz, float hx, float hy, float hz, const FastRay& f, float& tmin_out) {
  const float tx = __fmaf_rn(cx, f.mx, f.cx), ty = __fmaf_rn(cy, f.my, f.cy), tz = __fmaf_rn(cz, f.mz, f.cz);
  const float ex = fabsf(f.mx), ey = fabsf(f.my), ez = fabsf(f.mz);
  const float nx = __fmaf_rn(-hx, ex, tx), ny = __fmaf_rn(-hy, ey, ty), nz = __fmaf_rn(-hz, ez, tz);
  const float fx = __fmaf_rn(hx, ex, tx), fy = __fmaf_rn(hy, ey, ty), fz = __fmaf_rn(hz, ez, tz);
  const float tmax = fminf(fminf(fx, fy), fz);
  const float tmin = fmaxf(fmaxf(nx, ny), nz);
  tmin_out = tmin;
  return slab_verdict<SLACK>(tmin, tmax, f);
}
template <bool SLACK>
__device__ __forceinline__ bool slab_half(float ax, float ay, float az, float bx, float by, float bz, const FastRay& f, float& tmin_out) {
  return slab_fast<SLACK>(ax, ay, az, bx, by, bz, f, tmin_out);
}

__device__ __forceinline__ bool tri_test(F4 v0, F4 v1, F4 v2, const DRay& r, float& t_out, float& u_out, float& v_out) {
  const F4 v0v1 = v1 - v0;
  const F4 v0v2 = v2 - v0;
  const F4 n = cross(v0v1, v0v2);
  if (dot(r.d, n) > 0.0f) return false;
  const float denom = dot(n, n);
  const float ndd = dot(n, r.d);
  if (fabsf(ndd) < FLT_EPSILON) return false;
  const float d = -dot(n, v0);
  const float t = -(dot(n, to_vec(r.o)) + d) / ndd;
  if (t < 0.0f) return false;
  const F4 p = r.o + r.d * t;
  F4 c = cross(v1 - v0, to_vec(p - v0));
  if (dot(n, c) < 0.0f) return false;
  c = cross(v2 - v1, to_vec(p - v1));
  const float u = dot(n, c);
  if (u < 0.0f) return false;
  c = cross(v0 - v2, to_vec(p - v2));
  const float v = dot(n, c);
  if (v < 0.0f) return false;
  t_out = t;
  u_out = u / denom;
  v_out = v / denom;
  return true;
}

__device__ __forceinline__ DRay sphere_local_ray(const DevSphere& sp, const DRay& r) {
  F4 o = r.o + (-f4(sp.translation[0], sp.translation[1], sp.translation[2], 0.0f));
  F4 d = r.d;
  const F4 iq = f4(sp.inv_rotation[0], sp.inv_rotation[1], sp.inv_rotation[2], sp.inv_rotation[3]);
  d = rotate(d, iq);
  o = point_rotate(o, iq);
  o.w = 1.0f;
  const F4 is = f4(sp.inv_scale[0], sp.inv_scale[1], sp.inv_scale[2], sp.inv_scale[3]);
  d = d * is;
  o = point_scale(o, is);
  DRay l;
  l.o = o;
  l.d = d;
  l.rd = reciprocal(d);
  return l;
}
__device__ __forceinline__ bool sphere_test(const DevSphere& sp, const DRay& r, float& t_out) {
  const DRay l = sphere_local_ray(sp, r);
  const F4 center = f4(sp.center[0], sp.center[1], sp.center[2], sp.center[3]);
  const float a = dot(l.d, l.d);
  const F4 c_to_r = as_vec(l.o - center);
  const float b = dot(c_to_r, l.d);
  const float c = dot(c_to_r, c_to_r) - sp.radius2;
  const float det = b * b - a * c;
  if (det < 0.0f) return false;
  const float det_sqrt = sqrtf(det);
  const float t0 = (-b + det_sqrt) / a;
  const float t1 = (-b - det_sqrt) / a;
  if (t0 < 0.0f && t1 < 0.0f) return false;
  float t;
  if (t0 >= 0.0f && t1 >= 0.0f) t = fminf(t0, t1);
  else if (t0 >= 0.0f) t = t0;
  else t = t1;
  t_out = t;
  return true;
}

struct TriRecord {
  F4 v0, v1, v2;
  uint32_t rank, leaf;
};
constexpr uint32_t kTriQuads = 3, kTriFloats = 12;
__device__ __forceinline__ TriRecord load_tri(const DevScene& sc, uint32_t i) {
  const float4* p = sc.tris + (size_t)kTriQuads * i;
  const float4 q0 = p[0], q1 = p[1], q2 = p[2];
  TriRecord t;
  t.v0 = vec3(q0.x, q0.y, q0.z);
  t.v1 = vec3(q0.w, q1.x, q1.y);
  t.v2 = vec3(q1.z, q1.w, q2.x);
  t.rank = __float_as_uint(q2.y);
  t.leaf = __float_as_uint(q2.z);
  return t;
}

__device__ __forceinline__ bool tie_before(const DevScene& sc, uint32_t rank_a, uint32_t b) {
  if (b == RAYCA_NONE) return true;
  const uint32_t rank_b = __float_as_uint(reinterpret_cast<const float*>(sc.tris)[(size_t)kTriFloats * b + 9u]);
  return rank_a < rank_b;
}

__device__ __forceinline__ bool reference_candidate(const DevScene& sc, const TriRecord& t, const DRay& r) {
  if (!sc.ref_leaf_of) return true;
  const float4* b = sc.ref_leaf_boxes + 2ull * t.leaf;
  const float4 lo = b[0], hi = b[1];
  float tmin;
  return slab(lo.x, lo.y, lo.z, hi.x, hi.y, hi.z, r, tmin);
}

struct LaneCounters {
  uint32_t boxes, tris;
  unsigned long long slot_boxes, slot_tris;
  __device__ __forceinline__ bool books() const { return __lane_id() == (uint32_t)__ffsll((long long)__ballot(1)) - 1u; }
};

constexpr uint32_t kTerminated = 0x7FFFFFFFu;

template <bool SPILL>
struct NodeStack {
  uint32_t* lds;
  uint32_t* ovf;
  uint32_t gthread;
  uint32_t lds_entries, ovf_stride, sp;
  uint32_t top;
  __device__ __forceinline__ void clear() { sp = 0; top = kTerminated; }
#ifndef RAYCA_STACK_AS
#define RAYCA_STACK_AS 1
#endif
  typedef __attribute__((address_space(3))) uint32_t LdsWord;
  typedef __attribute__((address_space(1))) uint32_t GlobalWord;
  __device__ __forceinline__ void put(uint32_t i, uint32_t v) {
#if RAYCA_STACK_AS
    if (!SPILL || i < lds_entries) ((LdsWord*)lds)[i * kBlock] = v;
    else ((GlobalWord*)ovf)[(size_t)(i - lds_entries) * ovf_stride + gthread] = v;
#else
    if (!SPILL || i < lds_entries) lds[i * kBlock] = v;
    else ovf[(size_t)(i - lds_entries) * ovf_stride + gthread] = v;
#endif
  }
  __device__ __forceinline__ uint32_t get(uint32_t i) const {
#if RAYCA_STACK_AS
    uint32_t v;
    if (!SPILL || i < lds_entries) v = ((const LdsWord*)lds)[i * kBlock];
    else v = ((const GlobalWord*)ovf)[(size_t)(i - lds_entries) * ovf_stride + gthread];
    return v;
#else
    return (!SPILL || i < lds_entries) ? lds[i * kBlock] : ovf[(size_t)(i - lds_entries) * ovf_stride + gthread];
#endif
  }
  __device__ __forceinline__ void push(uint32_t v) {
    if (top != kTerminated) put(sp++, top);
    top = v;
  }
  __device__ __forceinline__ uint32_t pop() {
    const uint32_t r = top;
    if (sp == 0) top = kTerminated;
    else top = get(--sp);
    return r;
  }
  __device__ __forceinline__ void transfer(bool wr, bool rd, uint32_t at, bool keep, uint32_t v, uint32_t& out) {
    if (SPILL && __ballot(sp >= lds_entries) != 0ull) {
      const bool deep = at >= lds_entries;
      GlobalWord* const g = (GlobalWord*)ovf + ((size_t)(at - lds_entries) * ovf_stride + gthread);
      if (wr && deep) *g = top;
      if (rd && deep) {
        v = *g;
        asm volatile("" : "+v"(v));
        keep = false;
      }
      wr = wr && !deep;
      rd = rd && !deep;
    }
    if (wr) ((LdsWord*)lds)[at * kBlock] = top;
    asm volatile("" : "+v"(top), "+v"(out));
    top = keep ? top : v;
    if (rd) top = ((const LdsWord*)lds)[at * kBlock];
  }
  __device__ __forceinline__ void book(bool both, bool none, uint32_t far, uint32_t& cur) {
    const bool wr = both && top != kTerminated, rd = none && sp != 0u;
    const uint32_t at = rd ? sp - 1u : sp;
    transfer(wr, rd, at, !(both || none), both ? far : kTerminated, cur);
    sp = wr ? sp + 1u : at;
  }
  __device__ __forceinline__ uint32_t pop_late(bool take) {
    uint32_t r = take ? top : kTerminated;
    const bool rd = take && sp != 0u;
    sp -= rd ? 1u : 0u;
    transfer(false, rd, sp, !take, kTerminated, r);
    return r;
  }
};
template <bool SPILL>
__device__ __forceinline__ NodeStack<SPILL> make_stack(uint32_t* lds_base, const TraceLaunch& tl, uint32_t global_thread) {
  NodeStack<SPILL> st;
  st.lds = lds_base + rc_tid();
  st.ovf = tl.ovf;
  st.gthread = global_thread;
  st.lds_entries = tl.lds_entries;
  st.ovf_stride = tl.ovf_stride;
  st.clear();
  return st;
}

template <bool ORDERED, bool SPH, bool STATS, bool SLACK = true>
__device__ __forceinline__ void test_leaf(const DevScene& sc, const DRay& r, const FastRay& fr, uint32_t ref, float t_stop, DHit& hit, float& limit,
                                          LaneCounters& cnt) {
  const uint32_t first = ref & kLeafFirstMask;
  const uint32_t count = ((ref >> 25) & 63u) + 1u;
  for (uint32_t i = first; i < first + count; ++i) {
    const TriRecord tr = load_tri(sc, i);
    if (STATS) {
      cnt.tris++;
      if (cnt.books()) cnt.slot_tris += 64ull;
    }
    float t, u, v;
    bool got;
    if (SPH && tr.v0.x != tr.v0.x) {
      u = v = 0.0f;
      got = sphere_test(sc.spheres[__float_as_uint(tr.v0.y)], r, t);
    } else {
      got = tri_test(tr.v0, tr.v1, tr.v2, r, t, u, v);
    }
    if (got) {
      if ((t < hit.t || (t == hit.t && tie_before(sc, tr.rank, hit.prim))) && reference_candidate(sc, tr, r)) {
        hit.t = t;
        hit.prim = i;
        hit.u = u;
        hit.v = v;
        if (ORDERED) {
          limit = cull_limit<SLACK>(sc, fr, fminf(t, t_stop));
        }
      }
    }
  }
}

template <bool ORDERED, bool FAST, bool WIDE, bool SPILL, bool STATS, bool HALF, bool SLACK = true>
__device__ __forceinline__ uint32_t node_step(const DevScene& sc, const DRay& r, const FastRay& fr, float limit, uint32_t cur, NodeStack<SPILL>& st,
                                              LaneCounters& cnt) {
  if (STATS && cnt.books()) cnt.slot_boxes += WIDE ? 256ull : 128ull;
  if (WIDE) {
    float key[4];
    uint32_t ref[4];
    if (FAST && HALF) {
      const uint4* np = sc.nodes4_h + 4ull * cur;
      const uint4 q0 = np[0], q1 = np[1], q2 = np[2], q3 = np[3];
      if (STATS) cnt.boxes += 4;
      ref[0] = q3.x; ref[1] = q3.y; ref[2] = q3.z; ref[3] = q3.w;
      const float ax[4] = {lo16(q0.x), hi16(q0.x), lo16(q0.y), hi16(q0.y)}, ay[4] = {lo16(q0.z), hi16(q0.z), lo16(q0.w), hi16(q0.w)};
      const float az[4] = {lo16(q1.x), hi16(q1.x), lo16(q1.y), hi16(q1.y)}, bx[4] = {lo16(q1.z), hi16(q1.z), lo16(q1.w), hi16(q1.w)};
      const float by[4] = {lo16(q2.x), hi16(q2.x), lo16(q2.y), hi16(q2.y)}, bz[4] = {lo16(q2.z), hi16(q2.z), lo16(q2.w), hi16(q2.w)};
#pragma unroll
      for (int c = 0; c < 4; ++c) {
        float tc;
        bool h = slab_half<SLACK>(ax[c], ay[c], az[c], bx[c], by[c], bz[c], fr, tc);
        if (ORDERED) h = h && tc <= limit;
        key[c] = h ? (ORDERED ? tc : (float)c) : INFINITY;
      }
    } else {
    const float4* np = sc.nodes4 + 8ull * cur;
    const float4 lx = np[0], ly = np[1], lz = np[2], hx = np[3], hy = np[4], hz = np[5], cr = np[6];
    if (STATS) cnt.boxes += 4;
    ref[0] = __float_as_uint(cr.x); ref[1] = __float_as_uint(cr.y); ref[2] = __float_as_uint(cr.z); ref[3] = __float_as_uint(cr.w);
    const float ax[4] = {lx.x, lx.y, lx.z, lx.w}, ay[4] = {ly.x, ly.y, ly.z, ly.w}, az[4] = {lz.x, lz.y, lz.z, lz.w};
    const float bx[4] = {hx.x, hx.y, hx.z, hx.w}, by[4] = {hy.x, hy.y, hy.z, hy.w}, bz[4] = {hz.x, hz.y, hz.z, hz.w};
#pragma unroll
    for (int c = 0; c < 4; ++c) {
      float tc;
      bool h = FAST ? slab_fast<SLACK>(ax[c], ay[c], az[c], bx[c], by[c], bz[c], fr, tc) : slab(ax[c], ay[c], az[c], bx[c], by[c], bz[c], r, tc);
      if (ORDERED) h = h && tc <= limit;
      key[c] = h ? (ORDERED ? tc : (float)c) : INFINITY;
    }
    }
#define RC_CE(i, j)                                  \
  {                                                  \
const bool sw = key[i] > key[j];                 \
const float ka = sw ? key[j] : key[i];           \
const float kb = sw ? key[i] : key[j];           \
const uint32_t ra = sw ? ref[j] : ref[i];        \
const uint32_t rb = sw ? ref[i] : ref[j];        \
key[i] = ka; key[j] = kb; ref[i] = ra; ref[j] = rb; \
  }
    RC_CE(0, 1) RC_CE(2, 3) RC_CE(0, 2) RC_CE(1, 3) RC_CE(1, 2)
#undef RC_CE
    if (key[3] < INFINITY) st.push(ref[3]);
    if (key[2] < INFINITY) st.push(ref[2]);
    if (key[1] < INFINITY) st.push(ref[1]);
    cur = key[0] < INFINITY ? ref[0] : st.pop();
  } else {
    float tl, tr;
    bool hl, hr;
    uint32_t lref, rref;
    if (FAST && HALF) {
      const uint4* nh = sc.nodes_h + 2ull * cur;
      const uint4 a = nh[0], b = nh[1];
      hl = slab_half<SLACK>(lo16(a.x), hi16(a.x), lo16(a.y), hi16(a.y), lo16(a.z), hi16(a.z), fr, tl);
      hr = slab_half<SLACK>(lo16(a.w), hi16(a.w), lo16(b.x), hi16(b.x), lo16(b.y), hi16(b.y), fr, tr);
      lref = b.z;
      rref = b.w;
    } else {
      if (FAST && RAYCA_NODE_CH && RAYCA_NODE_CH48) {
        const float4* np = reinterpret_cast<const float4*>(reinterpret_cast<const char*>(sc.nodes_ch) + cur);
        const float4 q0 = np[0], q1 = np[1], q2 = np[2];
        hl = slab_ch<SLACK>(q0.x, q0.y, q0.z, q0.w, q1.x, q1.y, fr, tl);
        hr = slab_ch<SLACK>(q1.z, q1.w, q2.x, q2.y, q2.z, q2.w, fr, tr);
        lref = __builtin_amdgcn_perm(__float_as_uint(q1.x), __float_as_uint(q0.w), 0x05040100u);
        rref = __builtin_amdgcn_perm(__float_as_uint(q2.z), __float_as_uint(q2.y), 0x05040100u);
      } else {
        const float4* np = (FAST && RAYCA_NODE_CH ? sc.nodes_ch : sc.nodes) + 4ull * cur;
        const float4 q0 = np[0], q1 = np[1], q2 = np[2], q3 = np[3];
        if (FAST && RAYCA_NODE_CH) {
          hl = slab_ch<SLACK>(q0.x, q0.y, q0.z, q0.w, q1.x, q1.y, fr, tl);
          hr = slab_ch<SLACK>(q1.z, q1.w, q2.x, q2.y, q2.z, q2.w, fr, tr);
        } else if (FAST) {
          hl = slab_fast<SLACK>(q0.x, q0.y, q0.z, q0.w, q1.x, q1.y, fr, tl);
          hr = slab_fast<SLACK>(q1.z, q1.w, q2.x, q2.y, q2.z, q2.w, fr, tr);
        } else {
          hl = slab(q0.x, q0.y, q0.z, q0.w, q1.x, q1.y, r, tl);
          hr = slab(q1.z, q1.w, q2.x, q2.y, q2.z, q2.w, r, tr);
        }
        lref = __float_as_uint(q3.x);
        rref = __float_as_uint(q3.y);
      }
    }
    if (STATS) cnt.boxes += 2;
    if (ORDERED) {
      hl = hl && tl <= limit;
      hr = hr && tr <= limit;
    }
    if (hl && hr) {
      const bool left_first = !ORDERED || tl <= tr;
      st.push(left_first ? rref : lref);
      cur = left_first ? lref : rref;
    } else if (hl) {
      cur = lref;
    } else if (hr) {
      cur = rref;
    } else {
      cur = st.pop();
    }
  }
  return cur;
}

#ifndef RAYCA_LEAVE_K_CAMERA
#define RAYCA_LEAVE_K_CAMERA 0
#endif
#ifndef RAYCA_LEAVE_K_PATH0
#define RAYCA_LEAVE_K_PATH0 0
#endif
#ifndef RAYCA_LEAVE_K_BOUNCE
#define RAYCA_LEAVE_K_BOUNCE 8
#endif
template <bool ORDERED, bool FAST, bool SPH, bool WIDE, bool SPILL, bool STATS, bool HALF, int LEAVE_K, bool SLACK>
__device__ __forceinline__ bool trace_search(const DevScene& sc, const DRay& r, const FastRay& fr, float t_stop, NodeStack<SPILL>& st, DHit& hit, LaneCounters& cnt) {
  hit.t = INFINITY;
  hit.prim = RAYCA_NONE;
  hit.u = hit.v = 0.0f;
  float tmin;
  if (STATS) cnt.boxes++;
  uint32_t cur = WIDE ? sc.root_ref4 : (FAST && !HALF && RAYCA_NODE_CH ? sc.root_ref_ch : sc.root_ref);
  if (!slab(sc.root_min[0], sc.root_min[1], sc.root_min[2], sc.root_max[0], sc.root_max[1], sc.root_max[2], r, tmin)) cur = kTerminated;
  st.clear();
  const bool any_hit = ORDERED && t_stop < FLT_MAX;
  float limit = INFINITY;
  if (any_hit) limit = cull_limit<SLACK>(sc, fr, t_stop);
  if constexpr (LEAVE_K > 0) {
  for (;;) {
    for (;;) {
      const bool searching = !(cur & kLeafFlag) && cur != kTerminated;
      const uint32_t n = (uint32_t)__popcll(__ballot(searching));
      if (n == 0u) break;
      if (n < (uint32_t)LEAVE_K && __ballot((cur & kLeafFlag) != 0u) != 0ull) break;
      if (searching) cur = node_step<ORDERED, FAST, WIDE, SPILL, STATS, HALF, SLACK>(sc, r, fr, limit, cur, st, cnt);
    }
    if ((cur & kLeafFlag) && cur != kTerminated) {
      test_leaf<ORDERED, SPH, STATS, SLACK>(sc, r, fr, cur, t_stop, hit, limit, cnt);
      cur = (any_hit && hit.t < t_stop) ? kTerminated : st.pop();
    }
    if (__ballot(cur != kTerminated) == 0ull) break;
  }
  } else if constexpr (ORDERED && FAST && !WIDE && !HALF && RAYCA_NODE_CH && RAYCA_NODE_CH48) {
  while (cur != kTerminated) {
    if (!(cur & kLeafFlag)) {
      const float4* np = reinterpret_cast<const float4*>(reinterpret_cast<const char*>(sc.nodes_ch) + cur);
      float4 q0 = np[0], q1 = np[1], q2 = np[2];
      bool more;
      do {
        if (STATS && cnt.books()) cnt.slot_boxes += 128ull;
        float tl, tr;
        bool hl = slab_ch<SLACK>(q0.x, q0.y, q0.z, q0.w, q1.x, q1.y, fr, tl);
        bool hr = slab_ch<SLACK>(q1.z, q1.w, q2.x, q2.y, q2.z, q2.w, fr, tr);
        const uint32_t lref = __builtin_amdgcn_perm(__float_as_uint(q1.x), __float_as_uint(q0.w), 0x05040100u);
        const uint32_t rref = __builtin_amdgcn_perm(__float_as_uint(q2.z), __float_as_uint(q2.y), 0x05040100u);
        if (STATS) cnt.boxes += 2;
        hl = hl && tl <= limit;
        hr = hr && tr <= limit;
        const bool left_first = tl <= tr;
        const bool both = hl && hr, none = !(hl || hr);
        cur = none ? st.top : ((hl && (left_first || !hr)) ? lref : rref);
        more = !(cur & kLeafFlag) && cur != kTerminated;
        if (more) {
          const float4* nn = reinterpret_cast<const float4*>(reinterpret_cast<const char*>(sc.nodes_ch) + cur);
          q0 = nn[0]; q1 = nn[1]; q2 = nn[2];
        }
        st.book(both, none, left_first ? rref : lref, cur);
      } while (more);
    }
    if (cur != kTerminated) {
      test_leaf<ORDERED, SPH, STATS, SLACK>(sc, r, fr, cur, t_stop, hit, limit, cnt);
      cur = st.pop_late(!(any_hit && hit.t < t_stop));
    }
  }
  } else {
  while (cur != kTerminated) {
    while (!(cur & kLeafFlag) && cur != kTerminated) {
      cur = node_step<ORDERED, FAST, WIDE, SPILL, STATS, HALF, SLACK>(sc, r, fr, limit, cur, st, cnt);
    }
    if (cur != kTerminated) {
      test_leaf<ORDERED, SPH, STATS, SLACK>(sc, r, fr, cur, t_stop, hit, limit, cnt);
      if (any_hit && hit.t < t_stop) break;
      cur = st.pop();
    }
  }
  }
  return hit.prim != RAYCA_NONE;
}

constexpr int kSlackPerWave = 0, kSlackAlways = 1, kSlackNever = 2;
template <bool ORDERED, bool FAST, bool SPH, bool WIDE, bool SPILL, bool STATS, bool HALF = false, int LEAVE_K = 0, int SLACK_FORM = kSlackPerWave>
__device__ __forceinline__ bool trace(const DevScene& sc, const DRay& r, float t_stop, NodeStack<SPILL>& st, DHit& hit, LaneCounters& cnt) {
  const FastRay fr = make_fast(sc, r, HALF);
  if constexpr (!FAST || !RAYCA_RAY_SLACK || SLACK_FORM == kSlackNever) {
    return trace_search<ORDERED, FAST, SPH, WIDE, SPILL, STATS, HALF, LEAVE_K, false>(sc, r, fr, t_stop, st, hit, cnt);
  } else if constexpr (SLACK_FORM == kSlackAlways) {
    return trace_search<ORDERED, FAST, SPH, WIDE, SPILL, STATS, HALF, LEAVE_K, true>(sc, r, fr, t_stop, st, hit, cnt);
  } else {
    if (__ballot(ray_needs_slack(sc, r, fr)) != 0ull)
      return trace_search<ORDERED, FAST, SPH, WIDE, SPILL, STATS, HALF, LEAVE_K, true>(sc, r, fr, t_stop, st, hit, cnt);
    return trace_search<ORDERED, FAST, SPH, WIDE, SPILL, STATS, HALF, LEAVE_K, false>(sc, r, fr, t_stop, st, hit, cnt);
  }
}

__device__ __forceinline__ float query_bound(const QueryIo& q, uint32_t i, bool& dead) {
  const float tm = q.tmax ? q.tmax[i] : q.tmax_all;
  dead = !(tm > 0.0f);
  return tm < FLT_MAX ? tm : FLT_MAX;
}
__device__ __forceinline__ bool query_found(const DHit& hit, float bound) { return hit.prim != RAYCA_NONE && (bound == FLT_MAX || hit.t < bound); }
template <bool OCCLUDED>
__device__ __forceinline__ void query_store(const QueryIo& q, uint32_t i, const DHit& hit, bool found) {
  if (OCCLUDED) {
    q.occluded_out[i] = found ? 1 : 0;
  } else {
    if (q.t_out) q.t_out[i] = found ? hit.t : FLT_MAX;
    if (q.prim_out) q.prim_out[i] = found ? hit.prim : RAYCA_NONE;
    if (q.uv_out) {
      q.uv_out[2ull * i] = found ? hit.u : 0.0f;
      q.uv_out[2ull * i + 1ull] = found ? hit.v : 0.0f;
    }
  }
}

__device__ __forceinline__ Color load_color(const float* c) { return Color{c[0], c[1], c[2], c[3]}; }
__device__ __forceinline__ F4 load_vec3(const float* c) { return vec3(c[0], c[1], c[2]); }

__device__ __forceinline__ uint32_t f32_as_u32_sat(float v) {
  if (!(v == v) || v <= 0.0f) return 0u;
  if (v >= 4294967296.0f) return 0xFFFFFFFFu;
  return (uint32_t)v;
}
__device__ Color sample_texture(const DevScene& sc, uint32_t tex, F2 uv) {
  const DevTexture t = sc.textures[tex];
  const float fx = (uv.x - floorf(uv.x) + 1.0f) * (float)t.width;
  const float fy = (uv.y - floorf(uv.y) + 1.0f) * (float)t.height;
  const uint32_t x = f32_as_u32_sat(fx) % t.width, y = f32_as_u32_sat(fy) % t.height;
  const size_t idx = (size_t)y * t.width + x;
  const uint8_t* base = sc.image_bytes + t.byte_offset;
  if (t.color_type == RAYCA_COLOR_RGBA32F) {
    const float* f = reinterpret_cast<const float*>(base) + idx * 4;
    return Color{f[0] / 255.0f, f[1] / 255.0f, f[2] / 255.0f, f[3] / 255.0f};
  }
  if (t.color_type == RAYCA_COLOR_RGBA8) {
    const uint8_t* p = base + idx * 4;
    return Color{(float)p[0] / 255.0f, (float)p[1] / 255.0f, (float)p[2] / 255.0f, (float)p[3] / 255.0f};
  }
  const uint8_t* p = base + idx * 3;
  return Color{(float)p[0] / 255.0f, (float)p[1] / 255.0f, (float)p[2] / 255.0f, 255.0f / 255.0f};
}

__device__ __forceinline__ bool tex_valid(const DevScene& sc, uint32_t t) { return t != RAYCA_NONE && t < sc.texture_count; }

__device__ __forceinline__ Color pbr_color(const DevScene& sc, const DevMaterial& m, F2 uv) {
  const Color c = load_color(m.color);
  if (tex_valid(sc, m.albedo_texture)) return c * sample_texture(sc, m.albedo_texture, uv);
  return c;
}
__device__ __forceinline__ void pbr_metallic_roughness(const DevScene& sc, const DevMaterial& m, F2 uv, float& metallic, float& roughness) {
  if (tex_valid(sc, m.metallic_roughness_texture)) {
    const Color c = sample_texture(sc, m.metallic_roughness_texture, uv);
    metallic = c.b;
    roughness = c.r;
  } else {
    metallic = m.metallic_factor;
    roughness = m.roughness_factor;
  }
}
__device__ __forceinline__ DevMaterial default_material() {
  DevMaterial m{};
  m.color[0] = m.color[1] = m.color[2] = m.color[3] = 1.0f;
  m.ambient[3] = m.emission[3] = m.diffuse[3] = m.specular[3] = 1.0f;
  m.kind = RAYCA_MATERIAL_PBR;
  m.albedo_texture = m.normal_texture = m.metallic_roughness_texture = RAYCA_NONE;
  m.metallic_factor = 0.0f;
  m.roughness_factor = 1.0f;
  return m;
}

__device__ __forceinline__ F4 interp3(const float (*a)[3], float bu, float bv) {
  const float w2 = 1.0f - bu - bv;
  return (load_vec3(a[2]) * w2 + load_vec3(a[0]) * bu) + load_vec3(a[1]) * bv;
}

struct ShadeCtx {
  F4 point, normal, view, next_origin;
  Color kd, ks;
  float roughness, shininess;
  uint32_t kind;
};

#ifndef RAYCA_PARK_CTX
#define RAYCA_PARK_CTX 1
#endif
constexpr uint32_t kCtxQuads = 7;
__device__ __forceinline__ void park_ctx(float4* slot, const ShadeCtx& c) {
  slot[0 * kBlock] = make_float4(c.point.x, c.point.y, c.point.z, c.roughness);
  slot[1 * kBlock] = make_float4(c.normal.x, c.normal.y, c.normal.z, c.shininess);
  slot[2 * kBlock] = make_float4(c.view.x, c.view.y, c.view.z, __uint_as_float(c.kind));
  slot[3 * kBlock] = make_float4(c.kd.r, c.kd.g, c.kd.b, c.kd.a);
  slot[4 * kBlock] = make_float4(c.ks.r, c.ks.g, c.ks.b, c.ks.a);
}
__device__ __forceinline__ ShadeCtx unpark_ctx(const float4* slot) {
  const float4 q0 = slot[0 * kBlock], q1 = slot[1 * kBlock], q2 = slot[2 * kBlock], q3 = slot[3 * kBlock], q4 = slot[4 * kBlock];
  ShadeCtx c;
  c.point = f4(q0.x, q0.y, q0.z, 1.0f);
  c.normal = vec3(q1.x, q1.y, q1.z);
  c.view = vec3(q2.x, q2.y, q2.z);
  c.next_origin = c.point + c.normal * kRayBias;
  c.kd = Color{q3.x, q3.y, q3.z, q3.w};
  c.ks = Color{q4.x, q4.y, q4.z, q4.w};
  c.roughness = q0.w;
  c.shininess = q1.w;
  c.kind = __float_as_uint(q2.w);
  return c;
}

template <bool SPH>
__device__ __forceinline__ void shade_hit(const DevScene& sc, const DRay& ray, const DHit& hit, bool full, Color& color, bool& emissive,
                                          ShadeCtx& cx) {
  const PrimExt& e = sc.ext[hit.prim];
  const float bu = hit.u, bv = hit.v;
  const float w2 = 1.0f - bu - bv;
  const bool is_sphere = SPH && e.kind == RAYCA_GEOMETRY_SPHERE;
  const Color geom_color = is_sphere ? white() : (load_color(e.color[2]) * w2 + load_color(e.color[0]) * bu) + load_color(e.color[1]) * bv;
  const F2 uv = is_sphere ? F2{0.0f, 0.0f}
                          : F2{(e.uv[2][0] * w2 + e.uv[0][0] * bu) + e.uv[1][0] * bv, (e.uv[2][1] * w2 + e.uv[0][1] * bu) + e.uv[1][1] * bv};
  const DevMaterial m = (e.material != RAYCA_NONE && e.material < sc.material_count) ? sc.materials[e.material] : default_material();
  Color mc;
  if (m.kind == RAYCA_MATERIAL_PBR) mc = pbr_color(sc, m, uv);
  else if (m.kind == RAYCA_MATERIAL_PHONG) mc = load_color(m.ambient) + load_color(m.emission);
  else mc = load_color(m.diffuse);
  color = geom_color * mc;
  emissive = m.emissive != 0u;
  if (!full) return;
  F4 normal;
  F4 point = ray.o + ray.d * hit.t;
  F4 hit_dir = ray.d;
  if (is_sphere) {
    const DevSphere& sp = sc.spheres[e.node];
    const DRay l = sphere_local_ray(sp, ray);
    hit_dir = l.d;
    const F4 model_point = l.o + l.d * hit.t;
    const Trs wt{f4(sp.translation[0], sp.translation[1], sp.translation[2], 0.0f), f4(sp.rotation[0], sp.rotation[1], sp.rotation[2], sp.rotation[3]),
                 f4(sp.scale[0], sp.scale[1], sp.scale[2], 0.0f)};
    point = trs_apply_point(wt, model_point);
    const F4 hp = mat4_apply_point(reinterpret_cast<const float(*)[4]>(sp.inv_mat4), point);
    const F4 mn = normalized(as_vec(hp - f4(sp.center[0], sp.center[1], sp.center[2], sp.center[3])));
    const float* nm = sp.normal_mat;
    float out[3] = {0.0f, 0.0f, 0.0f};
    const float in[3] = {mn.x, mn.y, mn.z};
    for (int i = 0; i < 3; ++i)
      for (int j = 0; j < 3; ++j) out[i] += nm[4 * i + j] * in[j];
    normal = normalized(vec3(out[0], out[1], out[2]));
  } else {
    normal = normalized(interp3(e.normal, bu, bv));
  }
  if (!is_sphere && m.kind == RAYCA_MATERIAL_PBR && tex_valid(sc, m.normal_texture)) {
    const F4 tangent = normalized(interp3(e.tangent, bu, bv));
    const F4 bitangent = normalized(interp3(e.bitangent, bu, bv));
    F4 sn = premultiplied(sample_texture(sc, m.normal_texture, uv));
    sn = sn * 2.0f - f4(1.0f, 1.0f, 1.0f, 1.0f);
    normal = normalized(mat3_apply(mat3_tbn(tangent, bitangent, normal), sn));
  }
  cx.normal = normal;
  cx.point = point;
  cx.view = -hit_dir;
  cx.next_origin = cx.point + normal * kRayBias;
  cx.kind = m.kind;
  cx.shininess = m.shininess;
  if (m.kind == RAYCA_MATERIAL_PBR) {
    float me, ro;
    pbr_metallic_roughness(sc, m, uv, me, ro);
    const Color base = pbr_color(sc, m, uv);
    cx.kd = geom_color * base;
    cx.ks = me * base;
    cx.roughness = ro;
  } else {
    cx.kd = geom_color * load_color(m.diffuse);
    cx.ks = load_color(m.specular);
    cx.roughness = m.kind == RAYCA_MATERIAL_PHONG ? clampf(sqrtf(2.0f / (m.shininess + 2.0f)), 0.0f, 1.0f) : m.roughness_factor;
  }
}

#ifndef RAYCA_GGX_CLOSED_FORM
#define RAYCA_GGX_CLOSED_FORM 1
#endif
__device__ __forceinline__ float ggx_d(float a, F4 h, F4 n) {
  const float a2 = a * a;
  const float cos_theta = clampf(dot(h, n), 0.0f, 1.0f);
#if RAYCA_GGX_CLOSED_FORM
  const float q = a2 * (cos_theta * cos_theta) + (1.0f - cos_theta) * (1.0f + cos_theta);
  const float denominator = q * q;
  if (denominator == 0.0f || cos_theta == 0.0f) return 0.0f;
#else
  const float theta = acosf(cos_theta);
  const float denominator = powf(cos_theta, 4.0f) * powf(a2 + powf(tanf(theta), 2.0f), 2.0f);
  if (denominator == 0.0f) return 0.0f;
#endif
  return a2 * kFrac1Pi / denominator;
}
__device__ __forceinline__ float ggx_g1(float a, F4 omega, F4 n) {
  const float cos_theta = dot(omega, n);
  if (cos_theta <= 0.0f) return 0.0f;
#if RAYCA_GGX_CLOSED_FORM
  const float tan2 = cos_theta > 1.0f ? NAN : ((1.0f - cos_theta) * (1.0f + cos_theta)) / (cos_theta * cos_theta);
  return 2.0f / (1.0f + sqrtf(1.0f + a * a * tan2));
#else
  const float theta = acosf(cos_theta);
  return 2.0f / (1.0f + sqrtf(1.0f + a * a * powf(tanf(theta), 2.0f)));
#endif
}
__device__ __forceinline__ Color ggx_f(Color ks, F4 omega_i, F4 h) {
  const float oh = fabsf(dot(omega_i, h));
#if RAYCA_GGX_CLOSED_FORM
  const float x = 1.0f - oh, x2 = x * x;
  return ks + (white() - ks) * ((x2 * x2) * x);
#else
  return ks + (white() - ks) * powf(1.0f - oh, 5.0f);
#endif
}
__device__ __forceinline__ Color surf_brdf(const ShadeCtx& s, F4 omega_i) {
  if (s.kind == RAYCA_MATERIAL_PHONG) {
    const Color lambertian = s.kd * kFrac1Pi;
    const float sh = s.shininess;
    const F4 refl = normalized(reflect(-s.view, s.normal));
    const Color specular = (((s.ks * (sh + 2.0f)) * powf(dot(refl, omega_i), sh)) * kFrac1Pi) / 2.0f;
    return lambertian + specular;
  }
  Color bsdf = black();
  const F4 omega_o = s.view;
  const F4 n = s.normal;
  const float oin = clampf(dot(omega_i, n), 0.0f, 1.0f);
  const float oon = clampf(dot(omega_o, n), 0.0f, 1.0f);
  if (!(oin == 0.0f || oon == 0.0f)) {
    const float a = s.roughness;
    const F4 h = normalized(omega_i + omega_o);
    const Color f = ggx_f(s.ks, omega_i, h);
    const float g = ggx_g1(a, omega_i, n) * ggx_g1(a, omega_o, n);
    const float d = ggx_d(a, h, n);
    const float denominator = 4.0f * oin * oon;
    bsdf = ((f * g) * d) / denominator;
  }
  return s.kd * kFrac1Pi + bsdf;
}

__device__ __forceinline__ uint32_t xcc_id() {
  uint32_t v;
  asm volatile("s_getreg_b32 %0, hwreg(HW_REG_XCC_ID)" : "=s"(v));
  return v & 7u;
}
constexpr uint32_t kHeadStride = 64;
struct WorkCursor {
  uint32_t exhausted;
  uint32_t next, end;
};
__device__ __forceinline__ uint32_t next_batch(uint32_t* heads, uint32_t total, uint32_t home, WorkCursor& wc, uint32_t ticket) {
  if (wc.next < wc.end) return wc.next++;
  ticket = max(ticket, 1u);
  while (wc.exhausted < 8u) {
    const uint32_t part = (home + wc.exhausted) & 7u;
    const uint32_t lo = (uint32_t)(((uint64_t)part * total) >> 3), hi = (uint32_t)(((uint64_t)(part + 1u) * total) >> 3);
    uint32_t idx = 0;
    if (__lane_id() == 0) idx = atomicAdd(&heads[part * kHeadStride], ticket);
    idx = __builtin_amdgcn_readfirstlane(idx);
    if (idx < hi - lo) {
      wc.next = lo + idx + 1u;
      wc.end = min(lo + idx + ticket, hi);
      return lo + idx;
    }
    wc.exhausted++;
  }
  return RAYCA_NONE;
}

struct PathBuffers {
  float4* direct;
  float4* brdf;
  uint32_t* state;
  uint32_t npix;
};

__device__ __forceinline__ float4 as_f4(Color c) { return make_float4(c.r, c.g, c.b, c.a); }
__device__ __forceinline__ Color as_color(float4 c) { return Color{c.x, c.y, c.z, c.w}; }

__device__ __forceinline__ void finalize_pixel(const FrameParams& fp, Color acc, uint32_t p, uint8_t* rgba8, float4* rgba32f) {
  Color c = acc / (float)fp.spp;
  if (fp.inv_gamma != 1.0f) {
    c.r = powf(c.r, fp.inv_gamma);
    c.g = powf(c.g, fp.inv_gamma);
    c.b = powf(c.b, fp.inv_gamma);
  }
  if (rgba32f) rgba32f[p] = as_f4(c);
  if (rgba8) {
    const uint32_t packed = (uint32_t)quantize(c.r) | ((uint32_t)quantize(c.g) << 8) | ((uint32_t)quantize(c.b) << 16) | ((uint32_t)quantize(c.a) << 24);
    reinterpret_cast<uint32_t*>(rgba8)[p] = packed;
  }
}

__device__ __forceinline__ DRay camera_ray(const FrameParams& fp, uint32_t x, uint32_t y) {
  const float xx = (2.0f * ((((float)x + fp.sub_step_x) + fp.sub_offset) * fp.inv_width) - 1.0f) * fp.angle * fp.aspect;
  const float yy = (1.0f - 2.0f * ((((float)y + fp.sub_step_y) + fp.sub_offset) * fp.inv_height)) * fp.angle;
  F4 dir = normalized(vec3(xx, yy, -1.0f));
  F4 origin = point3(0.0f, 0.0f, 0.0f);
  dir = dir * fp.camera.scale;
  origin = point_scale(origin, fp.camera.scale);
  dir = rotate(dir, fp.camera.rotation);
  origin = point_rotate(origin, fp.camera.rotation);
  origin.w = 1.0f;
  origin = origin + fp.camera.translation;
  DRay r;
  r.o = origin;
  r.d = dir;
  r.rd = reciprocal(dir);
  return r;
}

__device__ __forceinline__ void push_ray(bool has, const QueuedRay& qr, QueuedRay* out, uint32_t* out_count) {
  const unsigned long long mask = __ballot(has);
  if (mask == 0ull) return;
  const uint32_t lane = __lane_id();
  const uint32_t leader = (uint32_t)__ffsll((long long)mask) - 1u;
  uint32_t base = 0;
  if (lane == leader) base = atomicAdd(out_count, (uint32_t)__popcll(mask));
  base = __shfl(base, (int)leader);
  if (has) out[base + (uint32_t)__popcll(mask & ((1ull << lane) - 1ull))] = qr;
}

constexpr int kModeFlat = 0, kModePath = 1, kModeGeneral = 2;

struct NeeSample {
  Color x;
  float t_stop;
  uint32_t quad;
};
__device__ __forceinline__ NeeSample nee_prepare(const DevScene& sc, const FrameParams& fp, const ShadeCtx& s, uint32_t li, uint32_t k,
                                                 uint32_t key, uint32_t& dim, DRay& shadow_ray) {
  const DevLight L = sc.lights[li];
  NeeSample ns;
  const F4 x_point = s.point;
  if (L.kind == RAYCA_LIGHT_POINT) {
    const F4 x1 = f4(L.position[0], L.position[1], L.position[2], L.position[3]);
    const F4 x_to_x1 = as_vec(x1 - x_point);
    const float dist = length(x_to_x1);
    const F4 omega = normalized(x_to_x1);
    shadow_ray = make_ray(s.next_origin, omega);
    const F4 dvec = to_vec(x_point) - to_vec(x1);
    const float r2 = norm2(dvec);
    const float rr = sqrtf(r2);
    const float fallof = hsum(f4(L.attenuation[0], L.attenuation[1], L.attenuation[2], 0.0f) * f4(1.0f, rr, r2, 0.0f));
    const Color le = (L.intensity * load_color(L.color)) / fallof;
    const Color brdf = surf_brdf(s, omega);
    const float r_squared = norm2(x_to_x1);
    const float d_omega = 1.0f / r_squared;
    const float n_dot_omega = clampf(dot(s.normal, omega), 0.0f, 1.0f);
    ns.x = ((le * brdf) * n_dot_omega) * d_omega;
    ns.t_stop = dist;
    ns.quad = 0u;
  } else {
    const F4 ab = f4(L.ab[0], L.ab[1], L.ab[2], 0.0f), ac = f4(L.ac[0], L.ac[1], L.ac[2], 0.0f);
    const float sc_f = (float)fp.strate_count;
    const float u1 = rng_f32(key, dim++) / sc_f;
    const float u2 = rng_f32(key, dim++) / sc_f;
    const F4 a = f4(L.position[0], L.position[1], L.position[2], L.position[3]);
    F4 x1 = (a + u1 * ab) + u2 * ac;
    if (fp.light_stratify) {
      const float i1 = (float)(k % fp.strate_count), i2 = (float)(k / fp.strate_count);
      x1 = x1 + ((ab / sc_f) * i1 + (ac / sc_f) * i2);
    }
    const F4 x_to_x1 = as_vec(x1 - x_point);
    const F4 omega = normalized(x_to_x1);
    shadow_ray = make_ray(s.next_origin, omega);
    const Color le = L.intensity * load_color(L.color);
    const Color brdf = surf_brdf(s, omega);
    const float r_squared = norm2(x_to_x1);
    const float d_omega = dot(f4(L.normal[0], L.normal[1], L.normal[2], 0.0f), omega) / r_squared;
    const float n_dot_omega = clampf(dot(s.normal, omega), 0.0f, 1.0f);
    ns.x = (((le * L.area) * brdf) * n_dot_omega) * d_omega;
    ns.t_stop = FLT_MAX;
    ns.quad = 1u;
  }
  return ns;
}

__device__ __forceinline__ bool nee_irrelevant(const NeeSample& ns) {
  return ns.x.r == 0.0f && ns.x.g == 0.0f && ns.x.b == 0.0f && fabsf(ns.x.a) < INFINITY;
}
constexpr uint32_t kShadowQuad = 1u, kShadowSkip = 2u;

struct WfBuffers {
  float4* hits;
  float4* sh_ray;
  float4* sh_x;
  uint32_t nls;
};

__device__ __forceinline__ bool tile_item_pixel(const FrameParams& fp, uint32_t item, uint32_t& x, uint32_t& r) {
  const uint32_t batch = item >> 6, j = item & 63u;
  if (batch >= fp.tile_count) return false;
  const uint32_t ty = batch / fp.tiles_x, tx = batch - ty * fp.tiles_x;
  x = tx * kTileW + (j & (kTileW - 1u));
  r = ty * kTileH + (j >> RAYCA_TILE_W_LOG2);
  return x < fp.width && r < fp.rows;
}
```

Measured before the change: 14060 Mrays/s.

## Shrink generation workgroup to one wave and read cold kernel args from kernarg

The generation kernel now launches with a configurable workgroup size, one wave by default instead of 256 threads, and the LDS stack stride, context parking and grid/ticket policy are sized to match. Kernel arguments are packed into a GenArgs struct, and rarely used fields are read directly from the kernarg segment instead of being held in SGPRs/VGPRs. The aim is to lower register pressure and allow finer-grained scheduling and occupancy for the persistent generation kernel. A variant library is also built with 4-wave blocks and cold args disabled for comparison. Single-wave blocks cost more workgroup launch overhead and change how LDS is allocated per CU.

```diff
diff --git a/__graft_entry__.py b/__graft_entry__.py
--- a/__graft_entry__.py
+++ b/__graft_entry__.py
@@ -8,6 +8,8 @@
 CSRC = os.path.join(ROOT, "rayca_amd", "csrc")
 LIB = os.path.join(CSRC, "librayca_hip.so")
 HIPCC = os.environ.get("HIPCC", "/opt/rocm/bin/hipcc")
+VARIANT_FLAGS = ["-DRAYCA_GEN_WAVES_PER_BLOCK=4", "-DRAYCA_COLD_ARGS=0"]
+VARIANT_LIB = os.path.join(CSRC, "variants", "librayca_gen_earlier.so")
 
 COMMON = ["-O3", "-std=c++17", "-fPIC", "-ffp-contract=off", "-fno-fast-math", "-Wall", "-Wno-unused-function",
           "-Wno-unused-result"]
@@ -24,7 +26,7 @@
     srcs = [os.path.join(CSRC, f) for f in ("kernels.hip", "refill.hip", "refill.hpp", "flavour.hpp", "trace_core.inc", "bvh_build.hip", "api.inc", "select.inc", "scene.inc", "post.inc", "aux_kernels.inc", "general.inc", "wavefront.inc", "surface.inc", "image_pass.inc", "denoise.inc", "denoise_variance.inc", "temporal.inc", "upsample.inc", "tonemap.inc",
                                             "host_scene.cpp", "host_scene.hpp", "device_types.hpp", "no_pk.hpp", "rayca_math.hpp", "staging.hpp", "libm_exact.hpp")]
     srcs.append(os.path.join(ROOT, "include", "rayca_hip.h"))
-    if force or _stale(LIB, srcs):
+    if force or _stale(LIB, srcs) or _stale(VARIANT_LIB, srcs):
         host_obj = os.path.join(CSRC, "host_scene.o")
         jobs = [subprocess.Popen(["g++", *COMMON, "-c", os.path.join(CSRC, "host_scene.cpp"), "-o", host_obj, "-pthread"])]
         objs = []
@@ -32,10 +34,14 @@
             obj = os.path.join(CSRC, unit + ".o")
             objs.append(obj)
             jobs.append(subprocess.Popen([HIPCC, "--offload-arch=gfx950", *COMMON, "-c", os.path.join(CSRC, unit + ".hip"), "-o", obj]))
+        os.makedirs(os.path.dirname(VARIANT_LIB), exist_ok=True)
+        variant_obj = os.path.join(os.path.dirname(VARIANT_LIB), "kernels_gen_earlier.o")
+        jobs.append(subprocess.Popen([HIPCC, "--offload-arch=gfx950", *COMMON, *VARIANT_FLAGS, "-c", os.path.join(CSRC, "kernels.hip"), "-o", variant_obj]))
         failed = [j.args for j in jobs if j.wait() != 0]
         if failed:
             raise subprocess.CalledProcessError(1, failed[0])
         subprocess.run([HIPCC, "--offload-arch=gfx950", "-shared", "-fPIC", *objs, host_obj, "-o", LIB, "-lpthread"], check=True)
+        subprocess.run([HIPCC, "--offload-arch=gfx950", "-shared", "-fPIC", variant_obj, *objs[1:], host_obj, "-o", VARIANT_LIB, "-lpthread"], check=True)
     subprocess.run(["make", "-s", "-C", os.path.join(ROOT, "oracle")], check=True)
     build_cpp_host()
     build_cpp_host("resident_draw")
diff --git a/rayca_amd/csrc/api.inc b/rayca_amd/csrc/api.inc
--- a/rayca_amd/csrc/api.inc
+++ b/rayca_amd/csrc/api.inc
@@ -611,7 +611,8 @@
   f.node_format |= (traits(tp.trav).wide ? (g == 0 ? 1u : 2u) : 0u) | (traits(tp.trav).half ? (g == 0 ? 4u : 8u) : 0u) | (ch.calibrating ? 256u : 0u) |
                    (ch.refill_cal ? 512u : 0u) | (ch.refill ? 1024u : 0u);
   const StackPlan sp = tp.stack;
-  const size_t lds_bytes = sp.lds_bytes + (park ? (size_t)kCtxQuads * 16u * kBlock : 0u);
+  const uint32_t block = ch.refill ? (uint32_t)kBlock : (uint32_t)kGenBlock;
+  const size_t lds_bytes = ((size_t)sp.lds_entries * 4u + (park ? (size_t)kCtxQuads * 16u : 0u)) * block;
   const bool sph = s->host.sphere_count != 0;
   GenKernel k = pick_kernel(f.plan.mode, g == 0, f.fused, tp.trav, sph, f.plan.stats);
   const RefillFlavour rf{tp.trav, sph, f.plan.stats};
@@ -619,17 +620,17 @@
   const uint32_t grid_mult = knobs().grid_mult;
   uint32_t grid = 0;
   TraceLaunch tl{};
-  int32_t rc = persistent_grid(s, ch.refill ? flat_refill_kernel(rf) : reinterpret_cast<const void*>(k), lds_bytes, batches, true, f.in_flight, grid_mult, grid);
-  if (rc != RAYCA_OK || (rc = bind_stack(c, sp, grid, tl)) != RAYCA_OK) return rc;
+  int32_t rc = persistent_grid(s, ch.refill ? flat_refill_kernel(rf) : reinterpret_cast<const void*>(k), lds_bytes, batches, true, f.in_flight, grid_mult, grid, block / 64u);
+  if (rc != RAYCA_OK || (rc = bind_stack(c, sp, grid, tl, block)) != RAYCA_OK) return rc;
   const uint32_t ticket_forced = knobs().ticket;
-  tl.ticket = ticket_forced ? ticket_forced : (batches >= 16u * grid ? 2u : 1u);
+  tl.ticket = ticket_forced ? ticket_forced : ticket_policy(batches, grid, block / 64u);
   size_t ev = 0;
   rc = timed_launch(f.log, f.stream, ch.refill ? RAYCA_KERNEL_FLAT_REFILL : RAYCA_KERNEL_GENERATION, f.timing || ch.calibrating || ch.refill_cal, true, [&] {
     if (ch.refill)
       launch_flat_refill(rf, grid, lds_bytes, f.stream, *f.dscene, f.fp, c->heads, f.rgba8, f.rgba32f, c->counters, tl);
     else
-      hipLaunchKernelGGL(k, dim3(grid), dim3(kBlock), lds_bytes, f.stream, *f.dscene, f.fp, c->heads, q.in, q.in_count, q.out, q.out_count, f.pb, g,
-                         f.rgba8, f.rgba32f, c->counters, tl);
+      hipLaunchKernelGGL(k, dim3(grid), dim3(kGenBlock), lds_bytes, f.stream,
+                         GenArgs{*f.dscene, f.fp, c->heads, q.in, q.in_count, q.out, q.out_count, f.pb, g, f.rgba8, f.rgba32f, c->counters, tl});
     return RAYCA_OK;
   }, &ev);
   if (rc != RAYCA_OK) return rc;
@@ -1024,6 +1025,7 @@
   int32_t rc = selftest_half_rounding(err);
   if (rc == RAYCA_OK) rc = selftest_device_layouts(err);
   if (rc == RAYCA_OK) rc = selftest_kernel_selection(err);
+  if (rc == RAYCA_OK) rc = selftest_grid_policy(err);
   return rc == RAYCA_OK ? RAYCA_OK : fail(rc, err);
 }
 
diff --git a/rayca_amd/csrc/kernels.hip b/rayca_amd/csrc/kernels.hip
--- a/rayca_amd/csrc/kernels.hip
+++ b/rayca_amd/csrc/kernels.hip
@@ -10,23 +10,46 @@
 RAYCA_NO_PK_BEGIN
 #include "trace_core.inc"
 
+#ifndef RAYCA_COLD_ARGS
+#define RAYCA_COLD_ARGS 1
+#endif
+struct GenArgs {
+  DevScene sc;
+  FrameParams fp;
+  uint32_t* heads;
+  const QueuedRay* in_rays;
+  const uint32_t* in_count;
+  QueuedRay* out_rays;
+  uint32_t* out_count;
+  PathBuffers pb;
+  uint32_t depth;
+  uint8_t* rgba8;
+  float4* rgba32f;
+  TraceCounters* counters;
+  TraceLaunch tl;
+};
+#if RAYCA_COLD_ARGS
+#define GEN_COLD(member) cold_arg<decltype(GenArgs::member)>((uint32_t)offsetof(GenArgs, member))
+#else
+#define GEN_COLD(member) (a.member)
+#endif
 template <int MODE, bool GEN0, bool ORDERED, bool FUSED, bool FAST, bool SPH, bool WIDE, bool SPILL, bool STATS, bool HALF>
-__global__ __launch_bounds__(kBlock, MODE == kModeFlat ? RAYCA_MIN_WAVES_FLAT : RAYCA_MIN_WAVES) void k_generation(DevScene sc, FrameParams fp, uint32_t* heads, const QueuedRay* in_rays,
-                                                       const uint32_t* in_count, QueuedRay* out_rays, uint32_t* out_count,
-                                                       PathBuffers pb, uint32_t depth, uint8_t* rgba8, float4* rgba32f,
-                                                       TraceCounters* counters, TraceLaunch tl) {
+__global__ __launch_bounds__(kGenBlock, MODE == kModeFlat ? RAYCA_MIN_WAVES_FLAT : RAYCA_MIN_WAVES) void k_generation(GenArgs a) {
+  const TraceLaunch& tl = a.tl;
+  uint32_t* const heads = a.heads;
+  const uint32_t depth = a.depth;
   extern __shared__ uint32_t lds_stack[];
-  NodeStack<SPILL> stack = make_stack<SPILL>(lds_stack, tl, rc_bid() * kBlock + rc_tid());
-  float4* const ctx_slot = reinterpret_cast<float4*>(lds_stack + tl.lds_entries * kBlock) + rc_tid();
+  NodeStack<SPILL, kGenBlock> stack = make_stack<SPILL, kGenBlock>(lds_stack, tl, rc_bid() * kGenBlock + rc_tid());
+  float4* const ctx_slot = reinterpret_cast<float4*>(lds_stack + tl.lds_entries * kGenBlock) + rc_tid();
   constexpr bool PARK = RAYCA_PARK_CTX && MODE == kModePath;
   const uint32_t lane = __lane_id();
   const uint32_t home = xcc_id();
   WorkCursor wc{};
-  const uint32_t total = GEN0 ? fp.tile_count : (*in_count + 63u) / 64u;
+  const uint32_t total = GEN0 ? GEN_COLD(fp).tile_count : (*GEN_COLD(in_count) + 63u) / 64u;
   LaneCounters cnt{};
   uint32_t n_shaded = 0, n_shadow = 0, n_bounce = 0;
-  const bool collect_emissive = GEN0 ? true : (fp.direct_sampler == RAYCA_SAMPLER_NONE);
-  const uint32_t nee_lights = (MODE == kModePath && fp.direct_sampler == RAYCA_SAMPLER_NEE) ? sc.light_count : 0u;
+  const bool collect_emissive = GEN0 ? true : (GEN_COLD(fp).direct_sampler == RAYCA_SAMPLER_NONE);
+  const uint32_t nee_lights = (MODE == kModePath && GEN_COLD(fp).direct_sampler == RAYCA_SAMPLER_NEE) ? GEN_COLD(sc).light_count : 0u;
 
   for (;;) {
     const uint32_t batch = next_batch(heads, total, home, wc, tl.ticket);
@@ -35,6 +58,7 @@
     uint32_t p = 0, key = 0;
     DRay ray;
     if (GEN0) {
+      const FrameParams& fp = GEN_COLD(fp);
       const uint32_t ty = batch / fp.tiles_x, tx = batch - ty * fp.tiles_x;
       const uint32_t x = tx * kTileW + (lane & (kTileW - 1u)), r = ty * kTileH + (lane >> RAYCA_TILE_W_LOG2);
       live = x < fp.width && r < fp.rows;
@@ -46,15 +70,15 @@
       }
     } else {
       const uint32_t i = batch * 64u + lane;
-      live = i < *in_count;
+      live = i < *GEN_COLD(in_count);
       if (live) {
-        const QueuedRay q = in_rays[i];
+        const QueuedRay q = GEN_COLD(in_rays)[i];
         ray = make_ray(point3(q.ox, q.oy, q.oz), vec3(q.dx, q.dy, q.dz));
         p = q.pixel;
         key = q.key;
       }
     }
-    const size_t slot = (size_t)depth * pb.npix + p;
+    const size_t slot = (size_t)depth * GEN_COLD(pb).npix + p;
     bool in_shadow = false;
     float t_stop = FLT_MAX;
     ShadeCtx cx;
@@ -68,17 +92,18 @@
       DHit hit;
       constexpr int kLeaveK = !ORDERED ? 0 : (MODE == kModeFlat ? RAYCA_LEAVE_K_CAMERA : (GEN0 ? RAYCA_LEAVE_K_PATH0 : RAYCA_LEAVE_K_BOUNCE));
       constexpr int kSlackForm = MODE == kModeFlat ? kSlackAlways : (GEN0 ? kSlackPerWave : kSlackNever);
-      const bool found = trace<ORDERED, FAST, SPH, WIDE, SPILL, STATS, HALF, kLeaveK, kSlackForm>(sc, ray, t_stop, stack, hit, cnt);
+      const bool found = trace<ORDERED, FAST, SPH, WIDE, SPILL, STATS, HALF, kLeaveK, kSlackForm>(a.sc, ray, t_stop, stack, hit, cnt);
       if (!in_shadow) {
         if (!found) {
           if (FUSED) direct = black() + black();
-          else pb.state[slot] = kVertexNone;
+          else GEN_COLD(pb).state[slot] = kVertexNone;
           live = false;
         } else {
           n_shaded++;
           Color color;
           bool emissive;
-          shade_hit<SPH>(sc, ray, hit, MODE == kModePath, color, emissive, cx);
+          const PathBuffers& pb = GEN_COLD(pb);
+          shade_hit<SPH>(GEN_COLD(sc), ray, hit, MODE == kModePath, color, emissive, cx);
           if (MODE == kModeFlat) {
             if (FUSED) direct = black() + color;
             else {
@@ -93,10 +118,10 @@
           } else {
             in_shadow = true;
             if (PARK) {
-              park_ctx(ctx_slot, cx);
+              park_ctx<kGenBlock>(ctx_slot, cx);
               float zero = 0.0f;
               asm volatile("" : "+v"(zero));
-              ctx_slot[6 * kBlock] = make_float4(zero, zero, zero, 1.0f);
+              ctx_slot[6 * kGenBlock] = make_float4(zero, zero, zero, 1.0f);
             }
           }
         }
@@ -105,6 +130,7 @@
         if (t_stop == FLT_MAX) {
           lit = false;
           if (found) {
+            const DevScene& sc = GEN_COLD(sc);
             const uint32_t hm = sc.ext[hit.prim].material;
             lit = hm != RAYCA_NONE && hm < sc.material_count && sc.materials[hm].emissive != 0u;
           }
@@ -112,12 +138,12 @@
           lit = !(found && hit.t < t_stop);
         }
         if (PARK) {
-          const Color sum = as_color(ctx_slot[6 * kBlock]) + (lit ? as_color(ctx_slot[5 * kBlock]) : black());
-          ctx_slot[6 * kBlock] = as_f4(sum);
+          const Color sum = as_color(ctx_slot[6 * kGenBlock]) + (lit ? as_color(ctx_slot[5 * kGenBlock]) : black());
+          ctx_slot[6 * kGenBlock] = as_f4(sum);
         } else {
           direct = direct + (lit ? ns_x : black());
         }
-        if (++k == fp.light_samples) {
+        if (++k == GEN_COLD(fp).light_samples) {
           k = 0;
           ++li;
         }
@@ -125,12 +151,13 @@
       if (live && in_shadow) {
         bool pending = false;
         while (li < nee_lights) {
-          if (PARK) cx = unpark_ctx(ctx_slot);
-          const NeeSample ns = nee_prepare(sc, fp, cx, li, k, key, dim, ray);
+          if (PARK) cx = unpark_ctx<kGenBlock>(ctx_slot);
+          const FrameParams& fp = GEN_COLD(fp);
+          const NeeSample ns = nee_prepare(GEN_COLD(sc), fp, cx, li, k, key, dim, ray);
           const bool irrelevant = ORDERED && nee_irrelevant(ns);
           if (STATS) {
             const unsigned long long m = __ballot(irrelevant);
-            if (m != 0ull && lane == (uint32_t)__ffsll((long long)m) - 1u) atomicAdd(&counters->nee_irrelevant, (unsigned long long)__popcll(m));
+            if (m != 0ull && lane == (uint32_t)__ffsll((long long)m) - 1u) atomicAdd(&GEN_COLD(counters)->nee_irrelevant, (unsigned long long)__popcll(m));
           }
           if (irrelevant && fp.nee_skip) {
             if (++k == fp.light_samples) {
@@ -139,7 +166,7 @@
             }
             continue;
           }
-          if (PARK) ctx_slot[5 * kBlock] = as_f4(ns.x);
+          if (PARK) ctx_slot[5 * kGenBlock] = as_f4(ns.x);
           else ns_x = ns.x;
           t_stop = ns.t_stop;
           pending = true;
@@ -152,8 +179,10 @@
       }
     }
     if (FUSED) {
-      if (has_pixel) finalize_pixel(fp, direct, p, rgba8, rgba32f);
+      if (has_pixel) finalize_pixel(GEN_COLD(fp), direct, p, GEN_COLD(rgba8), GEN_COLD(rgba32f));
     } else if (MODE == kModePath) {
+      const FrameParams& fp = GEN_COLD(fp);
+      const PathBuffers& pb = GEN_COLD(pb);
       bool want_bounce = false;
       QueuedRay next{};
       if (tail) {
@@ -168,8 +197,8 @@
           sdir = vec3(rc_cosf(omega_a) * st, rc_sinf(omega_a) * st, rc_cosf(theta));
         }
         if (PARK) {
-          cx = unpark_ctx(ctx_slot);
-          direct = as_color(ctx_slot[6 * kBlock]);
+          cx = unpark_ctx<kGenBlock>(ctx_slot);
+          direct = as_color(ctx_slot[6 * kGenBlock]);
         }
         pb.direct[slot] = as_f4(direct);
         if (depth < limit) {
@@ -198,7 +227,7 @@
       }
       n_shadow += (uint32_t)__popcll(__ballot(tail)) * nee_lights * fp.light_samples;
       n_bounce += (uint32_t)__popcll(__ballot(want_bounce));
-      push_ray(want_bounce, next, out_rays, out_count);
+      push_ray(want_bounce, next, GEN_COLD(out_rays), GEN_COLD(out_count));
     }
   }
   if (STATS) {
@@ -211,6 +240,7 @@
       stt += __shfl_down(stt, off);
     }
     if (lane == 0) {
+      TraceCounters* const counters = GEN_COLD(counters);
       atomicAdd(&counters->boxes, b);
       atomicAdd(&counters->tris, t);
       atomicAdd(&counters->shaded, sh);
@@ -221,6 +251,7 @@
   if (MODE == kModePath) {
     const unsigned long long s2 = n_shadow, b2 = n_bounce;
     if (lane == 0 && (s2 | b2)) {
+      TraceCounters* const counters = GEN_COLD(counters);
       atomicAdd(&counters->shadow, s2);
       atomicAdd(&counters->bounce, b2);
     }
diff --git a/rayca_amd/csrc/select.inc b/rayca_amd/csrc/select.inc
--- a/rayca_amd/csrc/select.inc
+++ b/rayca_amd/csrc/select.inc
@@ -11,8 +11,7 @@
 
 
 
-using GenKernel = void (*)(DevScene, FrameParams, uint32_t*, const QueuedRay*, const uint32_t*, QueuedRay*, uint32_t*, PathBuffers, uint32_t,
-                           uint8_t*, float4*, TraceCounters*, TraceLaunch);
+using GenKernel = void (*)(GenArgs);
 GenKernel pick_kernel(int mode, bool gen0, bool fused, Trav t, bool sph, bool stats) {
   const bool flat = mode == kModeFlat;
   return with_flavour([](auto T, auto FLAT, auto A, auto SPH, auto STATS) -> GenKernel {
@@ -76,11 +75,11 @@
   p.lds_bytes = (size_t)p.lds_entries * kBlock * 4u;
   return p;
 }
-int32_t bind_stack(FrameCtx* c, const StackPlan& sp, uint32_t grid, TraceLaunch& tl) {
+int32_t bind_stack(FrameCtx* c, const StackPlan& sp, uint32_t grid, TraceLaunch& tl, uint32_t block_threads = kBlock) {
   tl = TraceLaunch{};
   tl.lds_entries = sp.lds_entries;
   if (sp.spill_entries) {
-    tl.ovf_stride = grid * kBlock;
+    tl.ovf_stride = grid * block_threads;
     const int32_t rc = ensure(c->stack_spill, (size_t)sp.spill_entries * tl.ovf_stride * 4u);
     if (rc != RAYCA_OK) return rc;
     tl.ovf = static_cast<uint32_t*>(c->stack_spill.ptr);
@@ -228,14 +227,13 @@
   return RAYCA_OK;
 }
 
-int32_t persistent_grid(const RaycaScene* s, const void* kernel, size_t lds_bytes, uint32_t batches, bool capped, uint32_t in_flight,
-                        uint32_t per_cu_forced, uint32_t& grid) {
+uint32_t grid_policy(uint32_t regs, size_t lds_bytes, uint32_t batches, bool capped, uint32_t in_flight, uint32_t per_cu_forced, uint32_t cu_count,
+                     uint32_t block_waves) {
+  const uint32_t blocks_per_unit = 4u / block_waves;
   uint32_t per_cu = per_cu_forced;
   if (per_cu == 0) {
-    uint32_t regs = 0;
-    const int32_t rc = kernel_registers(kernel, regs);
-    if (rc != RAYCA_OK) return rc;
-    per_cu = std::min(512u / (((regs + 7u) / 8u) * 8u), lds_bytes ? (uint32_t)((160u * 1024u) / lds_bytes) : 8u);
+    const size_t unit_lds = lds_bytes * blocks_per_unit;
+    per_cu = std::min(512u / (((regs + 7u) / 8u) * 8u), unit_lds ? (uint32_t)((160u * 1024u) / unit_lds) : 8u);
     if (capped) {
       per_cu = std::max(1u, std::min(per_cu, 8u));
       if (in_flight >= 4u) per_cu = (per_cu + 1u) / 2u;
@@ -243,8 +241,65 @@
     }
     per_cu = std::max(1u, per_cu);
   }
-  const uint32_t need = (batches + 3u) / 4u;
-  grid = std::min((uint32_t)s->cu_count * per_cu, need ? need : 1u);
+  const uint32_t need = (batches + block_waves - 1u) / block_waves;
+  return std::min(cu_count * per_cu * blocks_per_unit, need ? need : 1u);
+}
+int32_t persistent_grid(const RaycaScene* s, const void* kernel, size_t lds_bytes, uint32_t batches, bool capped, uint32_t in_flight,
+                        uint32_t per_cu_forced, uint32_t& grid, uint32_t block_waves = 4u) {
+  uint32_t regs = 0;
+  if (per_cu_forced == 0) {
+    const int32_t rc = kernel_registers(kernel, regs);
+    if (rc != RAYCA_OK) return rc;
+  }
+  grid = grid_policy(regs, lds_bytes, batches, capped, in_flight, per_cu_forced, (uint32_t)s->cu_count, block_waves);
+  return RAYCA_OK;
+}
+uint32_t ticket_policy(uint32_t batches, uint32_t grid, uint32_t block_waves) { return batches >= 4u * block_waves * grid ? 2u : 1u; }
+
+int32_t selftest_grid_policy(std::string& err) {
+  struct Case { uint32_t regs; size_t wave_lds; uint32_t batches; bool capped; uint32_t in_flight, forced, waves; const char* what; };
+  constexpr uint32_t kCus = 256u, kPathLds = 12u * 256u + 7u * 1024u;
+  const Case cases[] = {
+      {125u, kPathLds, 32400u, true, 4u, 0u, 2048u, "the 1080p path frame, four in flight: 8 waves per CU"},
+      {125u, kPathLds, 32400u, true, 2u, 0u, 3072u, "the 1080p path frame, two in flight: 12 waves per CU"},
+      {125u, kPathLds, 32400u, true, 1u, 0u, 4096u, "the 1080p path frame alone: 16 waves per CU"},
+      {96u, 24u * 256u, 32400u, true, 1u, 0u, 5120u, "a Flat frame at 96 VGPRs: registers admit 5 waves per SIMD, LDS 6"},
+      {64u, 0u, 32400u, false, 1u, 0u, 8192u, "no LDS, uncapped: 8 waves per SIMD"},
+      {40u, 256u, 1u << 20, false, 1u, 0u, 12288u, "uncapped at 40 VGPRs and a little LDS: 12 waves per SIMD"},
+      {40u, 256u, 1u << 20, true, 1u, 0u, 8192u, "the same, capped: 8"},
+      {125u, kPathLds, 32400u, true, 4u, 3u, 3072u, "RAYCA_GRID_MULT=3 replaces the policy"},
+      {256u, 96u * 1024u, 32400u, true, 4u, 0u, 1024u, "a kernel nothing admits still gets one wave per SIMD"},
+  };
+  const auto fail_case = [&](const std::string& what) { err = "grid_policy: " + what; return RAYCA_ERR_BAD_ARG; };
+  for (const Case& c : cases)
+    for (uint32_t w : {1u, 2u, 4u}) {
+      const uint32_t grid = grid_policy(c.regs, c.wave_lds * w, c.batches, c.capped, c.in_flight, c.forced, kCus, w);
+      if (grid * w != c.waves) return fail_case(std::string(c.what) + ": " + std::to_string(grid) + " workgroups of " + std::to_string(w) + " waves, expected " + std::to_string(c.waves) + " waves");
+    }
+  const uint32_t small[][4] = {{0u, 1u, 1u, 1u}, {1u, 1u, 1u, 1u}, {6u, 6u, 3u, 2u}, {42u, 42u, 21u, 11u}, {2047u, 2047u, 1024u, 512u}};
+  for (const auto& r : small)
+    for (uint32_t i = 0; i < 3u; ++i)
+      if (const uint32_t grid = grid_policy(125u, kPathLds << i, r[0], true, 4u, 0u, kCus, 1u << i); grid != r[1 + i])
+        return fail_case(std::to_string(r[0]) + " batches in workgroups of " + std::to_string(1u << i) + " waves: " + std::to_string(grid) + " workgroups, expected " + std::to_string(r[1 + i]));
+  for (uint32_t regs : {24u, 64u, 96u, 125u, 128u, 200u})
+    for (uint32_t wave_lds : {0u, 1024u, 6144u, 10240u, 16384u})
+      for (uint32_t batches : {0u, 1u, 5u, 700u, 32400u, 129600u})
+        for (uint32_t in_flight : {1u, 2u, 3u, 4u, 8u})
+          for (int capped = 0; capped < 2; ++capped) {
+            const uint32_t w4 = grid_policy(regs, (size_t)wave_lds * 4u, 1u << 30, capped != 0, in_flight, 0u, kCus, 4u) * 4u;
+            for (uint32_t w : {1u, 2u, 4u}) {
+              const uint32_t full = grid_policy(regs, (size_t)wave_lds * w, 1u << 30, capped != 0, in_flight, 0u, kCus, w);
+              const uint32_t grid = grid_policy(regs, (size_t)wave_lds * w, batches, capped != 0, in_flight, 0u, kCus, w);
+              const std::string tuple = "(" + std::to_string(regs) + " VGPRs, " + std::to_string(wave_lds) + " B per wave, " + std::to_string(batches) + " batches, " +
+                                        std::to_string(in_flight) + " in flight, capped " + std::to_string(capped) + ", " + std::to_string(w) + " waves per workgroup)";
+              if (full * w != w4 || w4 % (4u * kCus) != 0u) return fail_case(tuple + ": " + std::to_string(full * w) + " waves fill the chip, " + std::to_string(w4) + " in 256-thread blocks");
+              if (grid == 0u || grid > full || (grid < full && grid != std::max(1u, (batches + w - 1u) / w))) return fail_case(tuple + ": " + std::to_string(grid) + " workgroups");
+            }
+          }
+  const uint32_t tickets[][4] = {{32400u, 2048u, 1u, 2u}, {32400u, 512u, 4u, 2u}, {32400u, 4096u, 1u, 2u}, {8192u, 2048u, 1u, 2u}, {8191u, 2048u, 1u, 1u}, {8191u, 512u, 4u, 1u}, {6u, 6u, 1u, 1u}};
+  for (const auto& t : tickets)
+    if (ticket_policy(t[0], t[1], t[2]) != t[3])
+      return fail_case("ticket_policy(" + std::to_string(t[0]) + " batches, " + std::to_string(t[1]) + " workgroups of " + std::to_string(t[2]) + " waves) is not " + std::to_string(t[3]));
   return RAYCA_OK;
 }
 
diff --git a/rayca_amd/csrc/trace_core.inc b/rayca_amd/csrc/trace_core.inc
--- a/rayca_amd/csrc/trace_core.inc
+++ b/rayca_amd/csrc/trace_core.inc
@@ -1,4 +1,10 @@
 constexpr int kBlock = 256;
+#ifndef RAYCA_GEN_WAVES_PER_BLOCK
+#define RAYCA_GEN_WAVES_PER_BLOCK 1
+#endif
+constexpr int kGenWaves = RAYCA_GEN_WAVES_PER_BLOCK;
+constexpr int kGenBlock = 64 * kGenWaves;
+static_assert(kGenWaves == 1 || kGenWaves == 2 || kGenWaves == 4, "k_generation's workgroup: 1, 2 or 4 waves");
 #ifndef RAYCA_TRACE_MIN_WAVES
 #define RAYCA_TRACE_MIN_WAVES 1
 #endif
@@ -13,6 +19,14 @@
 __device__ __forceinline__ uint32_t rc_bid() { return __builtin_amdgcn_workgroup_id_x(); }
 __device__ __forceinline__ uint32_t rc_bdim() { return __builtin_amdgcn_workgroup_size_x(); }
 __device__ __forceinline__ uint32_t rc_gdim() { return __builtin_amdgcn_grid_size_x() / __builtin_amdgcn_workgroup_size_x(); }
+
+template <class T>
+__device__ __forceinline__ const T& cold_arg(uint32_t offset) {
+  typedef __attribute__((address_space(4))) const char ConstByte;
+  ConstByte* p = (ConstByte*)__builtin_amdgcn_kernarg_segment_ptr();
+  asm volatile("" : "+s"(p));
+  return *(const T*)(p + offset);
+}
 
 struct DRay {
   F4 o, d, rd;
@@ -264,7 +278,7 @@
 
 constexpr uint32_t kTerminated = 0x7FFFFFFFu;
 
-template <bool SPILL>
+template <bool SPILL, int STRIDE = kBlock>
 struct NodeStack {
   uint32_t* lds;
   uint32_t* ovf;
@@ -279,21 +293,21 @@
   typedef __attribute__((address_space(1))) uint32_t GlobalWord;
   __device__ __forceinline__ void put(uint32_t i, uint32_t v) {
 #if RAYCA_STACK_AS
-    if (!SPILL || i < lds_entries) ((LdsWord*)lds)[i * kBlock] = v;
+    if (!SPILL || i < lds_entries) ((LdsWord*)lds)[i * STRIDE] = v;
     else ((GlobalWord*)ovf)[(size_t)(i - lds_entries) * ovf_stride + gthread] = v;
 #else
-    if (!SPILL || i < lds_entries) lds[i * kBlock] = v;
+    if (!SPILL || i < lds_entries) lds[i * STRIDE] = v;
     else ovf[(size_t)(i - lds_entries) * ovf_stride + gthread] = v;
 #endif
   }
   __device__ __forceinline__ uint32_t get(uint32_t i) const {
 #if RAYCA_STACK_AS
     uint32_t v;
-    if (!SPILL || i < lds_entries) v = ((const LdsWord*)lds)[i * kBlock];
+    if (!SPILL || i < lds_entries) v = ((const LdsWord*)lds)[i * STRIDE];
     else v = ((const GlobalWord*)ovf)[(size_t)(i - lds_entries) * ovf_stride + gthread];
     return v;
 #else
-    return (!SPILL || i < lds_entries) ? lds[i * kBlock] : ovf[(size_t)(i - lds_entries) * ovf_stride + gthread];
+    return (!SPILL || i < lds_entries) ? lds[i * STRIDE] : ovf[(size_t)(i - lds_entries) * ovf_stride + gthread];
 #endif
   }
   __device__ __forceinline__ void push(uint32_t v) {
@@ -319,10 +333,10 @@
       wr = wr && !deep;
       rd = rd && !deep;
     }
-    if (wr) ((LdsWord*)lds)[at * kBlock] = top;
+    if (wr) ((LdsWord*)lds)[at * STRIDE] = top;
     asm volatile("" : "+v"(top), "+v"(out));
     top = keep ? top : v;
-    if (rd) top = ((const LdsWord*)lds)[at * kBlock];
+    if (rd) top = ((const LdsWord*)lds)[at * STRIDE];
   }
   __device__ __forceinline__ void book(bool both, bool none, uint32_t far, uint32_t& cur) {
     const bool wr = both && top != kTerminated, rd = none && sp != 0u;
@@ -338,9 +352,9 @@
     return r;
   }
 };
-template <bool SPILL>
-__device__ __forceinline__ NodeStack<SPILL> make_stack(uint32_t* lds_base, const TraceLaunch& tl, uint32_t global_thread) {
-  NodeStack<SPILL> st;
+template <bool SPILL, int STRIDE = kBlock>
+__device__ __forceinline__ NodeStack<SPILL, STRIDE> make_stack(uint32_t* lds_base, const TraceLaunch& tl, uint32_t global_thread) {
+  NodeStack<SPILL, STRIDE> st;
   st.lds = lds_base + rc_tid();
   st.ovf = tl.ovf;
   st.gthread = global_thread;
@@ -383,8 +397,8 @@
   }
 }
 
-template <bool ORDERED, bool FAST, bool WIDE, bool SPILL, bool STATS, bool HALF, bool SLACK = true>
-__device__ __forceinline__ uint32_t node_step(const DevScene& sc, const DRay& r, const FastRay& fr, float limit, uint32_t cur, NodeStack<SPILL>& st,
+template <bool ORDERED, bool FAST, bool WIDE, bool SPILL, bool STATS, bool HALF, bool SLACK = true, int STRIDE = kBlock>
+__device__ __forceinline__ uint32_t node_step(const DevScene& sc, const DRay& r, const FastRay& fr, float limit, uint32_t cur, NodeStack<SPILL, STRIDE>& st,
                                               LaneCounters& cnt) {
   if (STATS && cnt.books()) cnt.slot_boxes += WIDE ? 256ull : 128ull;
   if (WIDE) {
@@ -500,8 +514,8 @@
 #ifndef RAYCA_LEAVE_K_BOUNCE
 #define RAYCA_LEAVE_K_BOUNCE 8
 #endif
-template <bool ORDERED, bool FAST, bool SPH, bool WIDE, bool SPILL, bool STATS, bool HALF, int LEAVE_K, bool SLACK>
-__device__ __forceinline__ bool trace_search(const DevScene& sc, const DRay& r, const FastRay& fr, float t_stop, NodeStack<SPILL>& st, DHit& hit, LaneCounters& cnt) {
+template <bool ORDERED, bool FAST, bool SPH, bool WIDE, bool SPILL, bool STATS, bool HALF, int LEAVE_K, bool SLACK, int STRIDE = kBlock>
+__device__ __forceinline__ bool trace_search(const DevScene& sc, const DRay& r, const FastRay& fr, float t_stop, NodeStack<SPILL, STRIDE>& st, DHit& hit, LaneCounters& cnt) {
   hit.t = INFINITY;
   hit.prim = RAYCA_NONE;
   hit.u = hit.v = 0.0f;
@@ -576,8 +590,8 @@
 }
 
 constexpr int kSlackPerWave = 0, kSlackAlways = 1, kSlackNever = 2;
-template <bool ORDERED, bool FAST, bool SPH, bool WIDE, bool SPILL, bool STATS, bool HALF = false, int LEAVE_K = 0, int SLACK_FORM = kSlackPerWave>
-__device__ __forceinline__ bool trace(const DevScene& sc, const DRay& r, float t_stop, NodeStack<SPILL>& st, DHit& hit, LaneCounters& cnt) {
+template <bool ORDERED, bool FAST, bool SPH, bool WIDE, bool SPILL, bool STATS, bool HALF = false, int LEAVE_K = 0, int SLACK_FORM = kSlackPerWave, int STRIDE = kBlock>
+__device__ __forceinline__ bool trace(const DevScene& sc, const DRay& r, float t_stop, NodeStack<SPILL, STRIDE>& st, DHit& hit, LaneCounters& cnt) {
   const FastRay fr = make_fast(sc, r, HALF);
   if constexpr (!FAST || !RAYCA_RAY_SLACK || SLACK_FORM == kSlackNever) {
     return trace_search<ORDERED, FAST, SPH, WIDE, SPILL, STATS, HALF, LEAVE_K, false>(sc, r, fr, t_stop, st, hit, cnt);
@@ -681,15 +695,17 @@
 #define RAYCA_PARK_CTX 1
 #endif
 constexpr uint32_t kCtxQuads = 7;
+template <int STRIDE = kBlock>
 __device__ __forceinline__ void park_ctx(float4* slot, const ShadeCtx& c) {
-  slot[0 * kBlock] = make_float4(c.point.x, c.point.y, c.point.z, c.roughness);
-  slot[1 * kBlock] = make_float4(c.normal.x, c.normal.y, c.normal.z, c.shininess);
-  slot[2 * kBlock] = make_float4(c.view.x, c.view.y, c.view.z, __uint_as_float(c.kind));
-  slot[3 * kBlock] = make_float4(c.kd.r, c.kd.g, c.kd.b, c.kd.a);
-  slot[4 * kBlock] = make_float4(c.ks.r, c.ks.g, c.ks.b, c.ks.a);
-}
+  slot[0 * STRIDE] = make_float4(c.point.x, c.point.y, c.point.z, c.roughness);
+  slot[1 * STRIDE] = make_float4(c.normal.x, c.normal.y, c.normal.z, c.shininess);
+  slot[2 * STRIDE] = make_float4(c.view.x, c.view.y, c.view.z, __uint_as_float(c.kind));
+  slot[3 * STRIDE] = make_float4(c.kd.r, c.kd.g, c.kd.b, c.kd.a);
+  slot[4 * STRIDE] = make_float4(c.ks.r, c.ks.g, c.ks.b, c.ks.a);
+}
+template <int STRIDE = kBlock>
 __device__ __forceinline__ ShadeCtx unpark_ctx(const float4* slot) {
-  const float4 q0 = slot[0 * kBlock], q1 = slot[1 * kBlock], q2 = slot[2 * kBlock], q3 = slot[3 * kBlock], q4 = slot[4 * kBlock];
+  const float4 q0 = slot[0 * STRIDE], q1 = slot[1 * STRIDE], q2 = slot[2 * STRIDE], q3 = slot[3 * STRIDE], q4 = slot[4 * STRIDE];
   ShadeCtx c;
   c.point = f4(q0.x, q0.y, q0.z, 1.0f);
   c.normal = vec3(q1.x, q1.y, q1.z);
```

Result: faster. 15490 Mrays/s, median of 6 (+10.1%).
